# aleju/face-generator

Measured on NVIDIA H100. Metric: 32x32 GAN train images/sec (1 D-iter + 1 G-iter per batch, batch 256/GPU), higher is better.
Workload: dtype f32

## Files before the change

face_generator_b200/csrc/convl.cu:

```cuda
#include "convl.h"

#include "k_conv_tc.h"
#include "k_misc.h"

int convl_dalloc(ConvLEnv& e, float** p, size_t elems) { return fg_dalloc(e.c, *e.allocs, p, elems); }

int ScalePairs::alloc(fg_ctx* c, std::vector<void*>& allocs, int pairs) {
  n = pairs;
  used = 0;
  return fg_dalloc(c, allocs, &base, 2 * (size_t)pairs);
}
int ScalePairs::take(float** pair) {
  if (used == n) {
    fg_set_error("a block of %d FP16 scale pairs is full", n);
    return FG_ERR_UNSUPPORTED;
  }
  *pair = base + 2 * used++;
  return FG_OK;
}
int ScalePairs::reset(fg_ctx* c) const {
  if (!tc_f16(c)) return FG_OK;
  FG_CUDA(cudaMemset2DAsync(base, 2 * sizeof(float), 0, sizeof(float), n, c->stream));
  return FG_OK;
}

namespace {
inline bool tc_f(const fg_ctx* c, const ConvL& L, int B) { return c->conv_impl != FG_CONV_SIMT && tc_conv_eligible(L.geom_k(B)); }
inline bool tc_d(const fg_ctx* c, const ConvL& L, int B) { return c->conv_impl != FG_CONV_SIMT && tc_conv_eligible(L.geom_d(B)); }
inline bool tc_w(const fg_ctx* c, const ConvL& L, int B) { return tc_f(c, L, B) && L.Cout % 128 == 0 && L.geom_k(B).Cin % 64 == 0; }
}

bool convl_tc_fwd(const fg_ctx* c, const ConvL& L) { return tc_f(c, L, 1); }
bool convl_tc_bwd(const fg_ctx* c, const ConvL& L) { return tc_f(c, L, 1) && tc_d(c, L, 1); }

int tc_op_split(fg_ctx* c, TcOp& op, const float* x, int64_t n, bool f16) {
  if (!f16) {
    if (op.split_ready) {
      op.split_ready = false;
      return FG_OK;
    }
    return tc_split(c, x, op.hi, op.lo, n);
  }
  if (op.amax_ready) op.amax_ready = false;
  else FG_TRY(tc_amax(c, x, n, op.s));
  return tc_split_h(c, x, op.hi, op.lo, n, op.s);
}

int convl_alloc(ConvLEnv& e, ConvL& L) {
  const size_t nw = (size_t)L.k * L.k * L.Cout * L.Cin;
  FG_TRY(convl_dalloc(e, &L.Wp, nw));
  FG_TRY(convl_dalloc(e, &L.Wpd, nw));
  if (L.nA) FG_TRY(convl_dalloc(e, &L.bp, L.Cout));
  if (!L.x.s) FG_TRY(convl_dalloc(e, &L.x.s, 2));
  if (!e.dy.s) FG_TRY(convl_dalloc(e, &e.dy.s, 2));
  if (tc_conv_eligible(L.geom_k(e.maxB))) {
    const int K = L.geom_k(e.maxB).Cin;
    const size_t nk = (size_t)L.k * L.k * L.Cout * K, nx = (size_t)e.maxB * L.H * L.H * K;
    FG_TRY(convl_dalloc(e, &L.Wf_hi, nk));
    FG_TRY(convl_dalloc(e, &L.Wf_lo, nk));
    FG_TRY(convl_dalloc(e, &L.x.hi, nx));
    FG_TRY(convl_dalloc(e, &L.x.lo, nx));
    if (L.kpad) {
      FG_TRY(convl_dalloc(e, &L.Wpad, nk));
      FG_TRY(convl_dalloc(e, &L.xpad, nx));
    }
  }
  if (L.need_dgrad && tc_conv_eligible(L.geom_d(e.maxB))) {
    FG_TRY(convl_dalloc(e, &L.Wd_hi, nw));
    FG_TRY(convl_dalloc(e, &L.Wd_lo, nw));
  }
  const int B = e.maxB;
  if (L.pad_out && !(tc_conv_eligible(ConvGeom{B, L.H, L.H, L.Cin, L.pad_out, L.k, 1}) &&
                     tc_conv_eligible(ConvGeom{B, L.H, L.H, L.pad_out, L.Cin, L.k, 1}) && L.Cin % 128 == 0))
    L.pad_out = 0;
  if (L.pad_dy && !(L.x.hi && tc_conv_eligible(ConvGeom{B, L.H, L.H, L.Cin, L.pad_dy, L.k, 1}) && L.Cin % 64 == 0))
    L.pad_dy = 0;
  if (L.pad_out) {
    const size_t nq = (size_t)L.k * L.k * L.pad_out * L.Cin;
    FG_TRY(convl_dalloc(e, &L.Wq_hi, nq));
    FG_TRY(convl_dalloc(e, &L.Wq_lo, nq));
    const size_t nx = (size_t)B * L.H * L.H * L.Cin;
    FG_TRY(convl_dalloc(e, &L.x.hi, nx));
    FG_TRY(convl_dalloc(e, &L.x.lo, nx));
  }
  return FG_OK;
}

int convl_pack(fg_ctx* c, ConvL& L, const float* P) {
  const int KK = L.k * L.k;
  const bool tc_on = c->conv_impl != FG_CONV_SIMT;
  const bool h = tc_on && tc_f16(c) && L.geom_k(1).Cin % 64 == 0 && (L.Cout % 64 == 0 || L.pad_out);
  L.packed_f16 = h;
  if (KK > 1 && tc_on && !L.nA && !L.cA && !L.pad_out && !L.kpad && L.Wf_hi && (L.Wd_hi || !L.need_dgrad) && tc_f(c, L, 1) &&
      (!L.need_dgrad || tc_d(c, L, 1))) {
    if (h) return tc_pack_split_h(c, P + L.w_off, L.Wf_hi, L.Wf_lo, L.Wd_hi, L.Wd_lo, L.Cout, L.Cin, KK);
    return tc_pack_split(c, P + L.w_off, L.Wf_hi, L.Wf_lo, L.Wd_hi, L.Wd_lo, L.Cout, L.Cin, KK);
  }
  FG_TRY(k_pack_weights(c, P + L.w_off, L.Wp, L.need_dgrad ? L.Wpd : nullptr, L.Cout, L.Cin, KK, L.nA, L.nS, L.cA, L.cS));
  if (L.bp) FG_TRY(k_pack_weights(c, P + L.b_off, L.bp, nullptr, L.Cout, 1, 1, L.nA, L.nS, 0, 0));
  if (!tc_on) return FG_OK;
  if (L.kpad && L.Wf_hi) {
    FG_CUDA(cudaMemcpy2DAsync(L.Wpad, L.kpad * sizeof(float), L.Wp, L.Cin * sizeof(float), L.Cin * sizeof(float), L.Cout,
                              cudaMemcpyDeviceToDevice, c->stream));
    if (h) return tc_split_h(c, L.Wpad, L.Wf_hi, L.Wf_lo, (int64_t)L.Cout * L.kpad);
    return tc_split(c, L.Wpad, L.Wf_hi, L.Wf_lo, (int64_t)L.Cout * L.kpad);
  }
  const int64_t nw = (int64_t)KK * L.Cout * L.Cin;
  if (h) {
    if (L.Wf_hi) FG_TRY(tc_split_h(c, L.Wp, L.Wf_hi, L.Wf_lo, nw));
    if (L.Wd_hi) FG_TRY(tc_split_h(c, L.Wpd, L.Wd_hi, L.Wd_lo, nw));
    if (L.pad_out) FG_TRY(k_pack_pad_split_h(c, P + L.w_off, L.Wq_hi, L.Wq_lo, L.Cout, L.pad_out, L.Cin, KK));
    return FG_OK;
  }
  if (L.Wf_hi) FG_TRY(tc_split(c, L.Wp, L.Wf_hi, L.Wf_lo, nw));
  if (L.Wd_hi) FG_TRY(tc_split(c, L.Wpd, L.Wd_hi, L.Wd_lo, nw));
  if (L.pad_out) FG_TRY(k_pack_pad_split(c, P + L.w_off, L.Wq_hi, L.Wq_lo, L.Cout, L.pad_out, L.Cin, KK));
  return FG_OK;
}

int convl_fwd(ConvLEnv& e, ConvL& L, const float* in, const float* P, float* out, int B) {
  fg_ctx* c = e.c;
  const ConvGeom g = L.geom(B);
  const float* bias = L.bp ? L.bp : P + L.b_off;
  const bool h = L.packed_f16;
  const float* os = h ? L.x.s + 1 : nullptr;
  if (L.pad_out && c->conv_impl != FG_CONV_SIMT) {
    FG_TRY(tc_op_split(c, L.x, in, (int64_t)B * L.H * L.H * L.Cin, h));
    {
      ScopedTimer t(c, L.tf);
      FG_TRY(tc_conv_fwd(c, L.x.hi, L.x.lo, L.Wq_hi, L.Wq_lo, nullptr, e.ga, ConvGeom{B, L.H, L.H, L.Cin, L.pad_out, L.k, 1}, 0,
                         nullptr, nullptr, h, os));
    }
    return k_compact_bias(c, e.ga, bias, out, (int64_t)B * L.H * L.H, L.Cout, L.pad_out);
  }
  if (tc_f(c, L, B)) {
    const ConvGeom gk = L.geom_k(B);
    if (L.kpad) {
      FG_CUDA(cudaMemcpy2DAsync(L.xpad, L.kpad * sizeof(float), in, L.Cin * sizeof(float), L.Cin * sizeof(float), (size_t)B * L.H * L.H,
                                cudaMemcpyDeviceToDevice, c->stream));
      in = L.xpad;
    }
    FG_TRY(tc_op_split(c, L.x, in, (int64_t)B * L.H * L.H * gk.Cin, h));
    ScopedTimer t(c, L.tf);
    return tc_conv_fwd(c, L.x.hi, L.x.lo, L.Wf_hi, L.Wf_lo, bias, out, gk, 0, nullptr, nullptr, h, os);
  }
  ScopedTimer t(c, L.tf);
  if (c->edge_impl && k_edge_eligible(g)) return k_conv_edge(c, in, L.Wp, bias, out, g);
  return k_small_eligible(g) ? k_conv_small(c, in, L.Wp, bias, out, g) : k_conv_simt(c, in, L.Wp, bias, out, g);
}

int convl_bwd(ConvLEnv& e, ConvL& L, const float* in, const float* dy, float* G, float* din, int B) {
  fg_ctx* c = e.c;
  const ConvGeom g = L.geom(B), gd = L.geom_d(B);
  const bool w_tc = G && tc_w(c, L, B), d_tc = din && tc_d(c, L, B);
  const bool h = L.packed_f16;
  float* sdy = L.sdy ? L.sdy : e.dy.s;
  const bool split_ready = e.dy.split_ready, amax_ready = e.dy.amax_ready, bias_ready = e.dy.bias_ready;
  e.dy.split_ready = e.dy.amax_ready = e.dy.bias_ready = false;
  const float *osy = h ? sdy + 1 : nullptr, *osx = h ? L.x.s + 1 : nullptr;
  const bool tc_on = c->conv_impl != FG_CONV_SIMT;
  const int64_t P = (int64_t)B * L.H * L.H;
  if (h && !amax_ready && (w_tc || d_tc || (G && tc_on && (L.pad_out || L.pad_dy)))) FG_TRY(tc_amax(c, dy, P * L.Cout, sdy));
  if (w_tc || d_tc) {
    if (h) FG_TRY(tc_split_h(c, dy, e.dy.hi, e.dy.lo, P * L.Cout, sdy));
    else if (!split_ready) FG_TRY(tc_split(c, dy, e.dy.hi, e.dy.lo, P * L.Cout));
  }
  if (G && tc_on && L.pad_out) {
    if (h) FG_TRY(k_pad_split_h(c, dy, e.pad.hi, e.pad.lo, P, L.Cout, L.pad_out, sdy));
    else FG_TRY(k_pad_split(c, dy, e.pad.hi, e.pad.lo, P, L.Cout, L.pad_out));
    {
      ScopedTimer t(c, L.tw);
      FG_TRY(tc_conv_wgrad(c, e.pad.hi, e.pad.lo, L.x.hi, L.x.lo, e.ws, ConvGeom{B, L.H, L.H, L.pad_out, L.Cin, L.k, 1}, h, osy, osx));
    }
    FG_TRY(k_unpack_wgrad_swapped(c, e.ws, G + L.w_off, L.Cout, L.pad_out, L.Cin, L.k * L.k));
    if (!bias_ready) FG_TRY(k_colsum_add(c, dy, G + L.b_off, P, L.Cout, 0, 0));
  } else if (G && tc_on && L.pad_dy && !w_tc) {
    if (h) FG_TRY(k_pad_split_h(c, dy, e.pad.hi, e.pad.lo, P, L.Cout, L.pad_dy, sdy));
    else FG_TRY(k_pad_split(c, dy, e.pad.hi, e.pad.lo, P, L.Cout, L.pad_dy));
    {
      ScopedTimer t(c, L.tw);
      FG_TRY(tc_conv_wgrad(c, L.x.hi, L.x.lo, e.pad.hi, e.pad.lo, e.ws, ConvGeom{B, L.H, L.H, L.Cin, L.pad_dy, L.k, 1}, h, osy, osx));
    }
    FG_TRY(k_unpack_wgrad_pad(c, e.ws, G + L.w_off, L.Cout, L.pad_dy, L.Cin, L.k * L.k));
    if (!bias_ready) FG_TRY(k_colsum_add(c, dy, G + L.b_off, P, L.Cout, 0, 0));
  } else if (G) {
    const int64_t koff = L.kpad && w_tc ? (int64_t)L.Cout * L.Cin : 0;
    {
      ScopedTimer t(c, L.tw);
      if (w_tc) FG_TRY(tc_conv_wgrad(c, L.x.hi, L.x.lo, e.dy.hi, e.dy.lo, e.ws + koff, L.geom_k(B), h, osy, osx));
      else if (k_small_eligible(g)) FG_TRY(k_wgrad_small(c, in, dy, e.ws, g));
      else FG_TRY(k_wgrad_simt(c, in, dy, e.ws, g));
    }
    if (koff)
      FG_CUDA(cudaMemcpy2DAsync(e.ws, L.Cin * sizeof(float), e.ws + koff, L.kpad * sizeof(float), L.Cin * sizeof(float), L.Cout,
                                cudaMemcpyDeviceToDevice, c->stream));
    FG_TRY(k_unpack_wgrad(c, e.ws, G + L.w_off, L.Cout, L.Cin, L.k * L.k, L.nA, L.nS, L.cA, L.cS));
    if (!bias_ready) FG_TRY(k_colsum_add(c, dy, G + L.b_off, P, L.Cout, L.nA, L.nS));
  }
  if (din) {
    ScopedTimer t(c, L.td);
    if (d_tc) return tc_conv_fwd(c, e.dy.hi, e.dy.lo, L.Wd_hi, L.Wd_lo, nullptr, din, gd, 0, nullptr, nullptr, h, osy);
    if (c->edge_impl && k_edge_eligible(gd)) return k_conv_edge(c, dy, L.Wpd, nullptr, din, gd);
    return k_small_eligible(gd) ? k_conv_small(c, dy, L.Wpd, nullptr, din, gd) : k_conv_simt(c, dy, L.Wpd, nullptr, din, gd);
  }
  return FG_OK;
}

bool upsl_tc(const fg_ctx* c, const UpsL& U) {
  return c->conv_impl != FG_CONV_SIMT && tc_conv_eligible(U.geom(1)) && U.Cout % 128 == 0 && U.Cin % 64 == 0;
}

int upsl_alloc(ConvLEnv& e, UpsL& U) {
  const size_t nw25 = (size_t)25 * U.Cout * U.Cin, nw36 = (size_t)36 * U.Cout * U.Cin;
  FG_TRY(convl_dalloc(e, &U.Wp, nw25));
  FG_TRY(convl_dalloc(e, &U.Wpd, nw25));
  FG_TRY(convl_dalloc(e, &U.Wf_hi, nw36));
  FG_TRY(convl_dalloc(e, &U.Wf_lo, nw36));
  FG_TRY(convl_dalloc(e, &U.Wd_hi, nw36));
  FG_TRY(convl_dalloc(e, &U.Wd_lo, nw36));
  FG_TRY(convl_dalloc(e, &U.Wx_hi, nw25));
  FG_TRY(convl_dalloc(e, &U.Wx_lo, nw25));
  const size_t nx = (size_t)e.maxB * (U.H / 2) * (U.H / 2) * U.Cin;
  FG_TRY(convl_dalloc(e, &U.x.hi, nx));
  FG_TRY(convl_dalloc(e, &U.x.lo, nx));
  if (!U.x.s) FG_TRY(convl_dalloc(e, &U.x.s, 2));
  return FG_OK;
}

int upsl_pack(fg_ctx* c, UpsL& U, const float* P) {
  const float* W = P + U.w_off;
  if (!upsl_tc(c, U)) return k_pack_weights(c, W, U.Wp, U.Wpd, U.Cout, U.Cin, 25, 0, 0, 0, 0);
  if (tc_f16(c)) FG_TRY(tc_pack_collapsed_h(c, W, U.Wf_hi, U.Wf_lo, U.Wd_hi, U.Wd_lo, U.Cout, U.Cin));
  else FG_TRY(tc_pack_collapsed(c, W, U.Wf_hi, U.Wf_lo, U.Wd_hi, U.Wd_lo, U.Cout, U.Cin));
  if (c->conv_impl == FG_CONV_TC_DENSE) FG_TRY(tc_pack_split(c, W, U.Wx_hi, U.Wx_lo, nullptr, nullptr, U.Cout, U.Cin, 25));
  return FG_OK;
}

int upsl_fwd(ConvLEnv& e, UpsL& U, const float* h, const float* P, float* z, int B, int* parts) {
  fg_ctx* c = e.c;
  const ConvGeom g = U.geom(B);
  const bool want = parts && *parts;
  if (parts) *parts = 0;
  const float* bias = P + U.b_off;
  if (!upsl_tc(c, U)) {
    ScopedTimer t(c, U.tf);
    return k_conv_simt(c, h, U.Wp, bias, z, g);
  }
  const bool f16 = tc_f16(c);
  FG_TRY(tc_op_split(c, U.x, h, (int64_t)B * (U.H / 2) * (U.H / 2) * U.Cin, f16));
  ScopedTimer t(c, U.tf);
  float* st = want && c->bn_epilogue ? c->bn_parts : nullptr;
  const bool dense = c->conv_impl == FG_CONV_TC_DENSE;
  return tc_conv_fwd(c, U.x.hi, U.x.lo, dense ? U.Wx_hi : U.Wf_hi, dense ? U.Wx_lo : U.Wf_lo, bias, z, g, dense ? 1 : 2, st,
                     st ? parts : nullptr, f16, f16 ? U.x.s + 1 : nullptr);
}

int upsl_bwd(ConvLEnv& e, UpsL& U, TcOp& dy, const float* h, const float* dz, float* G, float* dh, int B, bool* pooled) {
  fg_ctx* c = e.c;
  const ConvGeom g = U.geom(B);
  float* dW = G + U.w_off;
  *pooled = upsl_tc(c, U);
  if (!*pooled) {
    {
      ScopedTimer t(c, U.tw);
      FG_TRY(k_wgrad_simt(c, h, dz, e.ws, g));
    }
    FG_TRY(k_unpack_wgrad(c, e.ws, dW, U.Cout, U.Cin, 25, 0, 0, 0, 0));
    ScopedTimer t(c, U.td);
    return k_conv_simt(c, dz, U.Wpd, nullptr, dh, ConvGeom{B, U.H, U.H, U.Cout, U.Cin, 5, 1});
  }
  const bool f16 = tc_f16(c);
  FG_TRY(tc_op_split(c, dy, dz, (int64_t)B * U.H * U.H * U.Cout, f16));
  const float *sy = f16 ? dy.s + 1 : nullptr, *sx = f16 ? U.x.s + 1 : nullptr;
  if (f16 && U.tb && (c->bwd_merge == 2 ? tc_bwd_pair_eligible(c, g) : c->bwd_merge == 1 && tc_bwd_pair_pays(c, g))) {
    {
      ScopedTimer t(c, U.tb);
      FG_TRY(tc_conv_bwd_ups(c, U.x.hi, U.x.lo, dy.hi, dy.lo, U.Wd_hi, U.Wd_lo, e.ws, dh, g, sy, sx));
    }
    return tc_combine_collapsed_wgrad(c, e.ws, dW, U.Cout, U.Cin);
  }
  {
    ScopedTimer t(c, U.tw);
    FG_TRY(tc_conv_wgrad(c, U.x.hi, U.x.lo, dy.hi, dy.lo, e.ws, g, f16, sy, sx));
  }
  FG_TRY(tc_combine_collapsed_wgrad(c, e.ws, dW, U.Cout, U.Cin));
  ScopedTimer t(c, U.td);
  return tc_conv_dgrad_ups(c, dy.hi, dy.lo, U.Wd_hi, U.Wd_lo, dh, g, f16, sy);
}
```

face_generator_b200/csrc/convl.h:

```cpp
#pragma once
#include <vector>

#include "fg_internal.h"

inline bool tc_f16(const fg_ctx* c) { return c->mma_f16 && c->conv_impl == FG_CONV_TC_COLLAPSED; }

struct AmaxInto {
  fg_ctx* c;
  AmaxInto(fg_ctx* c_, TcOp& op) : AmaxInto(c_, op.s, &op.amax_ready) {}
  AmaxInto(fg_ctx* c_, float* pair, bool* done) : c(c_) {
    if (tc_f16(c)) {
      c->amax_out = reinterpret_cast<unsigned*>(pair);
      c->amax_done = done;
    }
  }
  ~AmaxInto() { c->amax_out = nullptr; }
};

int tc_op_split(fg_ctx* c, TcOp& op, const float* x, int64_t n, bool f16);

inline int pack_key(const fg_ctx* c) { return c->conv_impl | (c->mma_f16 << 4); }
int convl_dalloc(ConvLEnv& e, float** p, size_t elems);
int convl_alloc(ConvLEnv& e, ConvL& L);
bool convl_tc_fwd(const fg_ctx* c, const ConvL& L);
bool convl_tc_bwd(const fg_ctx* c, const ConvL& L);
int convl_pack(fg_ctx* c, ConvL& L, const float* P);
int convl_fwd(ConvLEnv& e, ConvL& L, const float* in, const float* P, float* out, int B);
int convl_bwd(ConvLEnv& e, ConvL& L, const float* in, const float* dy, float* G, float* din, int B);

bool upsl_tc(const fg_ctx* c, const UpsL& U);
int upsl_alloc(ConvLEnv& e, UpsL& U);
int upsl_pack(fg_ctx* c, UpsL& U, const float* P);
int upsl_fwd(ConvLEnv& e, UpsL& U, const float* h, const float* P, float* z, int B, int* parts = nullptr);
int upsl_bwd(ConvLEnv& e, UpsL& U, TcOp& dy, const float* h, const float* dz, float* G, float* dh, int B, bool* pooled);

int gen_alloc(ConvLEnv& e, UpsGen& G, const GenDesc& d);
int gen_pack(fg_ctx* c, UpsGen& G, NetPair& p);
int gen_forward(ConvLEnv& e, UpsGen& G, NetPair& p, const float* noise, int B, bool training);
int gen_backward(ConvLEnv& e, UpsGen& G, NetPair& p, const float* dy, float* dnoise);
void gen_debug_rows(const UpsGen& G, std::vector<DebugTensor>& rows);
```

face_generator_b200/csrc/fg_internal.h:

```cpp
#pragma once
#include <cuda_runtime.h>
#include <cstdint>
#include <cstdio>
#include <deque>
#include <functional>
#include <initializer_list>
#include <map>
#include <string>
#include <vector>

#include "fg_b200.h"

void fg_set_error(const char* fmt, ...);

#define FG_CUDA(call)                                                                               \
  do {                                                                                              \
    cudaError_t e__ = (call);                                                                       \
    if (e__ != cudaSuccess) {                                                                       \
      fg_set_error("%s:%d: %s -> %s", __FILE__, __LINE__, #call, cudaGetErrorString(e__));          \
      return FG_ERR_CUDA;                                                                           \
    }                                                                                               \
  } while (0)
#define FG_TRY(call)                  \
  do {                                \
    int r__ = (call);                 \
    if (r__ != FG_OK) return r__;     \
  } while (0)
#define FG_REQUIRE(cond, ...)         \
  do {                                \
    if (!(cond)) {                    \
      fg_set_error(__VA_ARGS__);      \
      return FG_ERR_INVALID;          \
    }                                 \
  } while (0)
#define LAUNCH_CHECK(c)                 \
  do {                                  \
    (c)->launches++;                    \
    FG_CUDA(cudaGetLastError());        \
  } while (0)
inline int grid_for(int64_t n, int block, int cap = 132 * 16) {
  int64_t g = (n + block - 1) / block;
  if (g > cap) g = cap;
  if (g < 1) g = 1;
  return (int)g;
}
#define GRID_STRIDE(i, n) \
  for (int64_t i = blockIdx.x * (int64_t)blockDim.x + threadIdx.x; i < (n); i += (int64_t)gridDim.x * blockDim.x)

constexpr int kMaskPerSample = 1984;
constexpr int kNoiseDim = 100;
constexpr int kSmallMaxParts = 2048;
constexpr int kGradTail = 8;
constexpr int kOptRedRows = 132 * 2;

struct ConvGeom {
  int B, H, W, Cin, Cout, k, ups;
};

struct GLayout {
  int64_t L1W, L1b, a1, C1W, C1b, g1, be1, a2, C2W, C2b, g2, be2, a3, C3W, C3b, total;
};
struct DLayout {
  int64_t cW[4], cb[4], ca[4], L1W, L1b, a5, L2W, L2b, a6, L3W, L3b, total;
};
GLayout make_g_layout(int C, int side);
DLayout make_d_layout(int C);

struct DeviceStats {
  float loss_D, loss_G;
  int conf[4];
  int trained_D;
  int t_D, t_G;
  float acc_D;
  int acc_count, acc_head;
  float step_D, step_G;
  int do_train_D, do_train_G;
};
constexpr int kAccHistMax = 1024;
constexpr int kBnState = 768;

struct StepGraph {
  std::vector<uint8_t> key;
  cudaGraphExec_t exec = nullptr;
  int64_t launches = 0;
  bool failed = false;
};

struct NetPair {
  int64_t nG = 0, nD = 0;
  float *PG = nullptr, *PD = nullptr, *gG = nullptr, *gD = nullptr;
  float *tailG = nullptr, *tailD = nullptr;
  float *mG = nullptr, *vG = nullptr, *mD = nullptr, *vD = nullptr;
  float* bnG = nullptr;
  DeviceStats* dstats = nullptr;
  DeviceStats* hstats = nullptr;
  float* acc_hist = nullptr;
  bool G_packed = false, D_packed = false;
  std::vector<StepGraph> graphs;
  const char* optim_timer[2] = {nullptr, nullptr};
};

struct ScalePairs {
  float* base = nullptr;
  int n = 0, used = 0;
  int alloc(fg_ctx* c, std::vector<void*>& allocs, int pairs);
  int take(float** pair);
  int reset(fg_ctx* c) const;
};

struct TcOp {
  float *hi = nullptr, *lo = nullptr;
  float* s = nullptr;
  bool split_ready = false, amax_ready = false, bias_ready = false;
};
struct ConvL {
  int Cin = 0, Cout = 0, k = 1, H = 1;
  int64_t w_off = 0, b_off = 0;
  int cA = 0, cS = 0;
  int nA = 0, nS = 0;
  float *Wp = nullptr, *Wpd = nullptr;
  float* bp = nullptr;
  float *Wf_hi = nullptr, *Wf_lo = nullptr, *Wd_hi = nullptr, *Wd_lo = nullptr;
  TcOp x;
  float* sdy = nullptr;
  int kpad = 0;
  float *xpad = nullptr, *Wpad = nullptr;
  bool packed_f16 = false;
  int pad_out = 0, pad_dy = 0;
  float *Wq_hi = nullptr, *Wq_lo = nullptr;
  bool need_dgrad = true;
  const char *tf = "", *td = "", *tw = "";
  ConvGeom geom(int B) const { return ConvGeom{B, H, H, Cin, Cout, k, 1}; }
  ConvGeom geom_k(int B) const { return ConvGeom{B, H, H, kpad ? kpad : Cin, Cout, k, 1}; }
  ConvGeom geom_d(int B) const { return ConvGeom{B, H, H, Cout, Cin, k, 1}; }
};

struct UpsL {
  int Cin = 0, Cout = 0, H = 0;
  int64_t w_off = 0, b_off = 0;
  float *Wp = nullptr, *Wpd = nullptr;
  float *Wf_hi = nullptr, *Wf_lo = nullptr, *Wd_hi = nullptr, *Wd_lo = nullptr;
  float *Wx_hi = nullptr, *Wx_lo = nullptr;
  TcOp x;
  const char *tf = "", *td = "", *tw = "", *tb = nullptr;
  ConvGeom geom(int B) const { return ConvGeom{B, H, H, Cin, Cout, 5, 2}; }
};

struct ConvLEnv {
  fg_ctx* c = nullptr;
  int maxB = 0;
  std::vector<void*>* allocs = nullptr;
  float *ga = nullptr;
  TcOp dy;
  TcOp pad;
  float* ws = nullptr;
};

struct GenDesc {
  int side;
  const char* prefix;
  int l1_kpad;
  bool bwd_merge;
};

struct UpsGen {
  int S = 32, C = 3;
  GLayout gl;
  ConvL GL1, GC3;
  UpsL GU[2];
  ScalePairs pairs;
  float* sdz[2] = {nullptr, nullptr};
  float *noise = nullptr, *z0 = nullptr, *h0 = nullptr, *z1 = nullptr, *h1 = nullptr, *z2 = nullptr, *h2 = nullptr,
        *z3 = nullptr, *y = nullptr;
  float *dz3 = nullptr, *dfull = nullptr, *dz2 = nullptr, *dz1 = nullptr, *dz0 = nullptr;
  float *bn_mean[2] = {nullptr, nullptr}, *bn_istd[2] = {nullptr, nullptr}, *bn_mg = nullptr;
  int B = 0;
  bool train = true, valid = false;
  int pack_key = -1;
  std::deque<std::string> names;
  const char *t_bn2_finalize = nullptr, *t_bn2_stats = nullptr, *t_bn2_apply = nullptr, *t_bn2_bwd_reduce = nullptr,
             *t_bn2_bwd_apply = nullptr;
};

struct TimerRec {
  double ms = 0;
  int64_t launches = 0;
  std::vector<std::pair<cudaEvent_t, cudaEvent_t>> pending;
};

struct fg_ctx {
  int device = 0, maxB = 0, C = 3;
  cudaStream_t stream = nullptr;
  bool own_stream = true;
  int64_t launches = 0;
  int conv_impl = FG_CONV_TC_COLLAPSED;
  int sm_count = 132;
  int opt_D = 0, opt_G = 0;
  float sgd_mom_D = 0.f, sgd_mom_G = 0.f;
  DLayout dl;
  std::vector<void*> allocs;
  NetPair net;
  float *ownPG = nullptr, *ownPD = nullptr, *ownGG = nullptr, *ownGD = nullptr;
  float* tail_sep = nullptr;
  float* small_ws = nullptr;
  float* wgrad_ws = nullptr;
  size_t wgrad_ws_elems = 0;
  float* splitk_ws = nullptr;
  size_t splitk_ws_elems = 0;
  double* red_ws = nullptr;
  size_t red_ws_elems = 0;
  double* red_ws_opt = nullptr;
  unsigned* red_ticket = nullptr;
  double* bn_slice_acc = nullptr;
  float* bn_parts = nullptr;
  int edge_impl = 1;
  int bn_epilogue = 1;
  int mma_f16 = 1;
  float* lop_sx = nullptr;
  float* lop_sy = nullptr;
  unsigned* amax_out = nullptr;
  bool* amax_done = nullptr;
  double* bn_acc = nullptr;
  int D_B = 0;
  bool D_train = true, D_fwd_valid = false;
  float *D_x = nullptr, *D_z[4] = {nullptr, nullptr, nullptr, nullptr}, *D_p[4] = {nullptr, nullptr, nullptr, nullptr};
  float *D_zl1 = nullptr, *D_hl1 = nullptr, *D_zl2 = nullptr, *D_hl2 = nullptr, *D_logit = nullptr, *D_out = nullptr;
  float* D_masks = nullptr;
  float D_drop_scale = 2.0f, D_spatial_eval = 0.8f;
  float *D_dlogit = nullptr, *D_dh = nullptr, *D_dzl = nullptr, *D_dz = nullptr, *D_dp = nullptr, *D_dx = nullptr;
  float* D_targets = nullptr;
  float* stage_pinned = nullptr;
  size_t stage_pinned_bytes = 0;
  float* io_dev = nullptr;
  size_t io_dev_elems = 0;
  float* io_dev2 = nullptr;
  float *in_real = nullptr, *in_noiseD = nullptr, *in_noiseG = nullptr, *in_masksD = nullptr, *in_masksG = nullptr;
  float* scratch[8] = {nullptr, nullptr, nullptr, nullptr, nullptr, nullptr, nullptr, nullptr};
  size_t scratch_elems[8] = {0, 0, 0, 0, 0, 0, 0, 0};
  void* nccl_comm = nullptr;
  int world = 1, rank = 0;
  int dp_overlap = 1;
  int reserve_sms = 0;
  int bwd_merge = 1, bwd_merge_ctas = 0;
  int* bwd_claim = nullptr;
  int use_graph = 1, graph_epoch = 0;
  uint64_t* seed_dev = nullptr;
  cudaStream_t comm_stream = nullptr;
  cudaEvent_t ev_fork = nullptr, ev_join = nullptr;
  bool debug_keep = false;
  int keep_B = 0;
  float* keep_D[8] = {nullptr, nullptr, nullptr, nullptr, nullptr, nullptr, nullptr, nullptr};
  cudaEvent_t events[16] = {};
  bool timing = false;
  std::map<std::string, TimerRec> timers;
  ConvLEnv env;
  UpsGen G;
  ConvL Dc[4], DL1, DL2;
  ScalePairs D_pairs;
};

struct ScopedTimer {
  fg_ctx* c;
  TimerRec* rec = nullptr;
  cudaEvent_t e0 = nullptr, e1 = nullptr;
  ScopedTimer(fg_ctx* c_, const char* name) : c(c_) {
    if (c->timing && name) {
      rec = &c->timers[name];
      cudaEventCreate(&e0);
      cudaEventCreate(&e1);
      cudaEventRecord(e0, c->stream);
    }
  }
  ~ScopedTimer() {
    if (rec) {
      cudaEventRecord(e1, c->stream);
      rec->pending.emplace_back(e0, e1);
    }
  }
};

int k_fill(fg_ctx* c, float* p, float v, int64_t n);
int k_nchw_to_nhwc(fg_ctx* c, const float* src, float* dst, int B, int C, int HW);
int k_nhwc_to_nchw(fg_ctx* c, const float* src, float* dst, int B, int C, int HW);
int k_pack_weights(fg_ctx* c, const float* W, float* Wp, float* Wpd, int N, int Cc, int KK, int nA, int nS, int cA,
                   int cS);
int k_unpack_wgrad(fg_ctx* c, const float* dWp, float* dW, int N, int Cc, int KK, int nA, int nS, int cA, int cS);
int k_colsum_add(fg_ctx* c, const float* X, float* out, int64_t P, int N, int nA, int nS);
int k_prelu_fwd(fg_ctx* c, const float* z, const float* slope, float* h, int64_t n);
int k_prelu_bwd(fg_ctx* c, const float* dh, const float* z, const float* slope, float* dz, float* dslope, int B, int H,
                int W, int C, int pool);
int k_bn_stats(fg_ctx* c, const float* z, double* acc2C, int64_t P, int C);
bool k_bn4_ok(int C);
int k_bn_stats4(fg_ctx* c, const float* z, double* acc, int64_t P, int C);
int k_bn_bwd_reduce4(fg_ctx* c, const float* dh, const float* z, const float* mean, const float* istd, const float* gamma,
                     const float* beta, const float* slope, double* acc, float* dslope, int64_t P, int C);
int k_bn_finalize(fg_ctx* c, double* acc2C, float* mean, float* istd, float* run_mean, float* run_var, int64_t P,
                  int C);
int k_bn_finalize_parts(fg_ctx* c, const float* part, int nparts, float* mean, float* istd, float* run_mean, float* run_var,
                        int64_t P, int C);
int k_bn_eval_prep(fg_ctx* c, const float* run_mean, const float* run_var, float* mean, float* istd, int C);
int k_bn_prelu_apply(fg_ctx* c, const float* z, const float* mean, const float* istd, const float* gamma,
                     const float* beta, const float* slope, float* h, int64_t P, int C, float* hi = nullptr,
                     float* lo = nullptr);
int k_bn_prelu_bwd_reduce(fg_ctx* c, const float* dh, const float* z, const float* mean, const float* istd,
                          const float* gamma, const float* beta, const float* slope, double* acc2C, float* dslope,
                          int B, int H, int W, int C, int pool);
int k_bn_bwd_finalize(fg_ctx* c, double* acc2C, float* mg2C, float* dgamma, float* dbeta, int64_t P, int C);
int k_bn_prelu_bwd_apply(fg_ctx* c, const float* dh, const float* z, const float* mean, const float* istd,
                         const float* gamma, const float* beta, const float* slope, const float* mg2C, float* dz,
                         int B, int H, int W, int C, int pool, float* hi = nullptr, float* lo = nullptr,
                         float* dbias = nullptr);
int k_sigmoid_fwd(fg_ctx* c, const float* z, float* y, int64_t n);
int k_sigmoid_bwd(fg_ctx* c, const float* dy, const float* y, float* dz, int64_t n);
int k_masks_generate(fg_ctx* c, float* masks, int B, uint64_t seed, float p_spatial, float p_drop,
                     const uint64_t* seed_dev = nullptr);
int k_set_u64(fg_ctx* c, uint64_t* dst, uint64_t v);
int k_d_act_pool_fwd(fg_ctx* c, const float* z, const float* slope, const float* masks, int moff, float eval_scale,
                     float* p, int B, int H, int W, int C, float* hi = nullptr, float* lo = nullptr);
int k_d_act_pool_bwd(fg_ctx* c, const float* dp, const float* z, const float* slope, const float* masks, int moff,
                     float eval_scale, float* dz, float* dslope, int B, int H, int W, int C, float* hi = nullptr,
                     float* lo = nullptr, float* dbias = nullptr);
int k_lin_act_drop_fwd(fg_ctx* c, const float* z, const float* slope, const float* masks, int moff, float scale,
                       float* h, int B, int N);
int k_lin_act_drop_bwd(fg_ctx* c, const float* dh, const float* z, const float* slope, const float* masks, int moff,
                       float scale, float* dz, float* dslope, int B, int N);
int k_sigmoid_bce(fg_ctx* c, const float* logit, float* out, float* dlogit, float* loss_out, float* tail4, int B,
                  int n_ones);
int k_bce_fwd(fg_ctx* c, const float* x, const float* t, int n, float* loss_out);
int k_bce_bwd(fg_ctx* c, const float* x, const float* t, int n, float* dx);
int k_sigmoid_grad_mul(fg_ctx* c, const float* dout, const float* out, float* dlogit, int n);
int k_penalty_loss(fg_ctx* c, const float* p, int64_t n, float l1, float l2, float* loss_inout);
int k_gate_and_prep(fg_ctx* c, DeviceStats* st, float* acc_hist, int net, const fg_hyper* h, const float* tail4, int B,
                    float world);
int k_gemv_fwd(fg_ctx* c, const float* x, const float* w, const float* bias, float* out, int B, int K);
int k_gemv_dgrad(fg_ctx* c, const float* dy, const float* w, float* dx, int B, int K);
int k_gemv_wgrad_add(fg_ctx* c, const float* x, const float* dy, float* dw, float* db, int B, int K);
int k_adam(fg_ctx* c, float* p, const float* g, float* m, float* v, int64_t n, float beta1, float beta2, float eps,
           float l1_grad, float l2, float clampv, float grad_scale, const float* step_dev, const int* flag_dev,
           float step_host, float* g_out);
int k_optim_update(fg_ctx* c, int mode, float* p, float* g, float* m, float* v, int64_t n, float beta1, float beta2, float eps,
                   float mom, float l1_grad, float l2, float clampv, float grad_scale, const float* step_dev,
                   const int* flag_dev, const int* t_dev);

int k_conv_simt(fg_ctx* c, const float* in, const float* Wp, const float* bias, float* out, ConvGeom g);
int k_wgrad_simt(fg_ctx* c, const float* in, const float* dY, float* dWp, ConvGeom g);
bool k_small_eligible(const ConvGeom& g);
int k_conv_small(fg_ctx* c, const float* in, const float* Wp, const float* bias, float* out, ConvGeom g);
int k_wgrad_small(fg_ctx* c, const float* in, const float* dY, float* dWp, ConvGeom g);

bool k_edge_eligible(const ConvGeom& g);
int k_conv_edge(fg_ctx* c, const float* in, const float* Wp, const float* bias, float* out, ConvGeom g);

inline int red_check(fg_ctx* c, int64_t rows, int64_t n) {
  if (rows * n > (int64_t)c->red_ws_elems) {
    fg_set_error("ordered reduction of %lld x %lld partials exceeds its workspace", (long long)rows, (long long)n);
    return FG_ERR_UNSUPPORTED;
  }
  return FG_OK;
}
int k_splitk_reduce(fg_ctx* c, const float* parts, int splits, int64_t n, float* out);

int tc_init(fg_ctx* c);
void tc_destroy(fg_ctx* c);

int net_alloc(fg_ctx* c);
void net_free(fg_ctx* c);
int net_pack_D(fg_ctx* c);
int net_D_forward(fg_ctx* c, const float* x_nhwc, int B, bool training, const fg_hyper* h);
int net_D_backward(fg_ctx* c, const float* dlogit_dev, bool want_wgrad, bool want_dx);
int net_train_step(fg_ctx* c, const fg_hyper* h, int B, const float* real_nchw_dev, const float* noiseD_dev,
                   const float* noiseG_dev, const float* masksD_dev, const float* masksG_dev, uint64_t seed,
                   bool allow_graph = false);
int net_allreduce(fg_ctx* c, float* buf, int64_t n);
int net_broadcast(fg_ctx* c, void* buf, size_t bytes);
int net_group(bool start);

int fg_dalloc(fg_ctx* c, std::vector<void*>& allocs, float** p, size_t n);
int pair_alloc(fg_ctx* c, std::vector<void*>& allocs, NetPair& p, int64_t nG, int64_t nD, bool bn);
void pair_clear_graphs(NetPair& p);
void pair_free(NetPair& p);
int pair_zero_grads(fg_ctx* c, NetPair& p, int net);
int pair_allreduce_grads(fg_ctx* c, NetPair& p, int net);
int pair_gate(fg_ctx* c, NetPair& p, int net, const fg_hyper* h, int B, float world);
int pair_optim(fg_ctx* c, NetPair& p, int net, const fg_hyper* h, float grad_scale);
int pair_broadcast(fg_ctx* c, NetPair& p);
int pair_step_stats(fg_ctx* c, const NetPair& p, fg_step_stats* stats);
int pair_set_params(fg_ctx* c, NetPair& p, int net, const float* src);
int pair_get_params(fg_ctx* c, const NetPair& p, int net, float* dst);
int pair_get_grads(fg_ctx* c, const NetPair& p, int net, float* dst);
int pair_set_adam_state(fg_ctx* c, NetPair& p, int net, const float* m, const float* v, int t);
int pair_get_adam_state(fg_ctx* c, const NetPair& p, int net, float* m, float* v, int* t);
int pair_set_bn_state(fg_ctx* c, NetPair& p, const float* src);
int pair_get_bn_state(fg_ctx* c, const NetPair& p, float* dst);
int net_graph_run(fg_ctx* c, NetPair& p, int B, const fg_hyper* h, std::initializer_list<const void*> inputs, uint64_t seed,
                  const std::function<int()>& body, bool allow_graph);

bool fg_is_dev(const void* p);
int fg_to_dev(fg_ctx* c, const float* p, size_t n, float* staging, const float** out);
int fg_to_user(fg_ctx* c, float* dst, const float* src_dev, size_t n);
struct DebugTensor {
  const char* name;
  const float* p;
  int64_t per;
  int B;
};
int64_t debug_tensor_copy(fg_ctx* c, const char* what, const DebugTensor* ents, size_t n_ents, const char* name, float* dst,
                          int64_t max_elems);

int dataset_check_feed(const fg_dataset* d, const fg_ctx* c, const char* what);
int dataset_draw_gather(fg_dataset* d, uint64_t seed, int B, int size, float* out_dev);
int dataset_draw_gather_c2f(fg_dataset* d, uint64_t seed, int B, int coarse_size, float* fine, float* coarse, float* diff);
int noise_uniform_dev(fg_ctx* c, uint64_t seed, int64_t n, float* out_dev);
```

face_generator_b200/csrc/gen.cu:

```cuda
#include "convl.h"

GLayout make_g_layout(int C, int side) {
  const int64_t n0 = 128 * (side / 4) * (side / 4);
  GLayout L;
  int64_t o = 0;
  L.L1W = o; o += n0 * kNoiseDim;
  L.L1b = o; o += n0;
  L.a1 = o; o += 1;
  L.C1W = o; o += 256 * 128 * 25;
  L.C1b = o; o += 256;
  L.g1 = o; o += 256;
  L.be1 = o; o += 256;
  L.a2 = o; o += 1;
  L.C2W = o; o += 128 * 256 * 25;
  L.C2b = o; o += 128;
  L.g2 = o; o += 128;
  L.be2 = o; o += 128;
  L.a3 = o; o += 1;
  L.C3W = o; o += (int64_t)C * 128 * 9;
  L.C3b = o; o += C;
  L.total = o;
  return L;
}

int gen_alloc(ConvLEnv& e, UpsGen& G, const GenDesc& d) {
  fg_ctx* c = e.c;
  const int S = d.side, C = c->C;
  G.S = S;
  G.C = C;
  G.gl = make_g_layout(C, S);
  const GLayout& gl = G.gl;
  auto timer = [&](const char* name) {
    G.names.push_back(std::string(d.prefix) + name);
    return G.names.back().c_str();
  };
  FG_TRY(G.pairs.alloc(c, *e.allocs, 8));
  ConvL& L1 = G.GL1;
  L1.Cin = kNoiseDim; L1.Cout = 128 * (S / 4) * (S / 4); L1.k = 1; L1.H = 1;
  L1.w_off = gl.L1W; L1.b_off = gl.L1b;
  L1.nA = 128; L1.nS = (S / 4) * (S / 4);
  L1.kpad = d.l1_kpad;
  L1.tf = timer("G.L1.fwd"); L1.td = timer("G.L1.dgrad"); L1.tw = timer("G.L1.wgrad");
  ConvL& C3 = G.GC3;
  C3.Cin = 128; C3.Cout = C; C3.k = 3; C3.H = S;
  C3.w_off = gl.C3W; C3.b_off = gl.C3b;
  C3.tf = timer("G.C3.fwd"); C3.td = timer("G.C3.dgrad"); C3.tw = timer("G.C3.wgrad");
  for (ConvL* L : {&L1, &C3}) {
    FG_TRY(G.pairs.take(&L->x.s));
    FG_TRY(G.pairs.take(&L->sdy));
    FG_TRY(convl_alloc(e, *L));
  }
  static const char* uf[2] = {"G.C1.fwd", "G.C2.fwd"};
  static const char* ud[2] = {"G.C1.dgrad", "G.C2.dgrad"};
  static const char* uw[2] = {"G.C1.wgrad", "G.C2.wgrad"};
  static const char* ub[2] = {"G.C1.wgrad+dgrad", "G.C2.wgrad+dgrad"};
  const int ci[2] = {128, 256}, co[2] = {256, 128}, hs[2] = {S / 2, S};
  const int64_t wo[2] = {gl.C1W, gl.C2W}, bo[2] = {gl.C1b, gl.C2b};
  for (int i = 0; i < 2; ++i) {
    UpsL& U = G.GU[i];
    U.Cin = ci[i]; U.Cout = co[i]; U.H = hs[i];
    U.w_off = wo[i]; U.b_off = bo[i];
    U.tf = timer(uf[i]); U.td = timer(ud[i]); U.tw = timer(uw[i]);
    U.tb = d.bwd_merge ? timer(ub[i]) : nullptr;
    FG_TRY(G.pairs.take(&U.x.s));
    FG_TRY(G.pairs.take(&G.sdz[i]));
    FG_TRY(upsl_alloc(e, U));
  }
  G.t_bn2_finalize = timer("G.bn2.finalize");
  G.t_bn2_stats = timer("hbm.G.bn2.stats");
  G.t_bn2_apply = timer("hbm.G.bn2.apply");
  G.t_bn2_bwd_reduce = timer("hbm.G.bn2.bwd_reduce");
  G.t_bn2_bwd_apply = timer("hbm.G.bn2.bwd_apply");
  const size_t B = e.maxB, n0 = L1.Cout, n1 = (size_t)256 * (S / 2) * (S / 2), n2 = (size_t)128 * S * S, n3 = (size_t)C * S * S;
  for (auto [p, n] : {std::pair<float**, size_t>{&G.noise, kNoiseDim}, {&G.z0, n0}, {&G.h0, n0}, {&G.z1, n1}, {&G.h1, n1},
                      {&G.z2, n2}, {&G.h2, n2}, {&G.z3, n3}, {&G.y, n3}, {&G.dz3, n3},
                      {&G.dfull, (size_t)256 * S * S},
                      {&G.dz2, n2}, {&G.dz1, n1}, {&G.dz0, n0}})
    FG_TRY(convl_dalloc(e, p, B * n));
  for (int i = 0; i < 2; ++i) {
    FG_TRY(convl_dalloc(e, &G.bn_mean[i], co[i]));
    FG_TRY(convl_dalloc(e, &G.bn_istd[i], co[i]));
  }
  return convl_dalloc(e, &G.bn_mg, 512);
}

int gen_pack(fg_ctx* c, UpsGen& G, NetPair& p) {
  if (p.G_packed && G.pack_key == pack_key(c)) return FG_OK;
  FG_TRY(convl_pack(c, G.GL1, p.PG));
  for (int i = 0; i < 2; ++i) FG_TRY(upsl_pack(c, G.GU[i], p.PG));
  FG_TRY(convl_pack(c, G.GC3, p.PG));
  p.G_packed = true;
  G.pack_key = pack_key(c);
  return FG_OK;
}

namespace {
int bn_stats(fg_ctx* c, UpsGen& G, NetPair& p, int i, const float* z, int B, bool training, int parts, const char* t_finalize,
             const char* t_stats) {
  const int Cc = G.GU[i].Cout;
  const int64_t P = (int64_t)B * G.GU[i].H * G.GU[i].H;
  float *rm = p.bnG + (i == 0 ? 0 : 512), *rv = rm + Cc;
  if (!training) return k_bn_eval_prep(c, rm, rv, G.bn_mean[i], G.bn_istd[i], Cc);
  if (parts) {
    ScopedTimer tm(c, t_finalize);
    return k_bn_finalize_parts(c, c->bn_parts, parts, G.bn_mean[i], G.bn_istd[i], rm, rv, P, Cc);
  }
  {
    ScopedTimer tm(c, t_stats);
    FG_TRY(k_bn_stats(c, z, c->bn_acc, P, Cc));
  }
  return k_bn_finalize(c, c->bn_acc, G.bn_mean[i], G.bn_istd[i], rm, rv, P, Cc);
}
}

int gen_forward(ConvLEnv& e, UpsGen& G, NetPair& p, const float* noise, int B, bool training) {
  fg_ctx* c = e.c;
  FG_REQUIRE(B >= 1 && B <= e.maxB, "G forward: batch %d out of range [1,%d]", B, e.maxB);
  FG_TRY(gen_pack(c, G, p));
  const GLayout& L = G.gl;
  const float* P = p.PG;
  const int S = G.S;
  if (noise != G.noise)
    FG_CUDA(cudaMemcpyAsync(G.noise, noise, sizeof(float) * B * kNoiseDim, cudaMemcpyDeviceToDevice, c->stream));
  G.B = B;
  G.train = training;
  FG_TRY(G.pairs.reset(c));
  FG_TRY(convl_fwd(e, G.GL1, G.noise, P, G.z0, B));
  {
    AmaxInto am(c, G.GU[0].x);
    FG_TRY(k_prelu_fwd(c, G.z0, P + L.a1, G.h0, (int64_t)B * G.GL1.Cout));
  }
  int parts = training ? 1 : 0;
  FG_TRY(upsl_fwd(e, G.GU[0], G.h0, P, G.z1, B, &parts));
  FG_TRY(bn_stats(c, G, p, 0, G.z1, B, training, parts, nullptr, nullptr));
  UpsL& C2 = G.GU[1];
  C2.x.split_ready = training && upsl_tc(c, C2) && !tc_f16(c);
  {
    AmaxInto am(c, C2.x);
    FG_TRY(k_bn_prelu_apply(c, G.z1, G.bn_mean[0], G.bn_istd[0], P + L.g1, P + L.be1, P + L.a2, G.h1,
                            (int64_t)B * (S / 2) * (S / 2), 256, C2.x.split_ready ? C2.x.hi : nullptr,
                            C2.x.split_ready ? C2.x.lo : nullptr));
  }
  parts = training ? 1 : 0;
  FG_TRY(upsl_fwd(e, C2, G.h1, P, G.z2, B, &parts));
  FG_TRY(bn_stats(c, G, p, 1, G.z2, B, training, parts, G.t_bn2_finalize, G.t_bn2_stats));
  {
    ScopedTimer tm(c, G.t_bn2_apply);
    FG_TRY(k_bn_prelu_apply(c, G.z2, G.bn_mean[1], G.bn_istd[1], P + L.g2, P + L.be2, P + L.a3, G.h2, (int64_t)B * S * S, 128));
  }
  FG_TRY(convl_fwd(e, G.GC3, G.h2, P, G.z3, B));
  FG_TRY(k_sigmoid_fwd(c, G.z3, G.y, (int64_t)B * S * S * G.C));
  G.valid = true;
  return FG_OK;
}

int gen_backward(ConvLEnv& e, UpsGen& G, NetPair& p, const float* dy, float* dnoise) {
  fg_ctx* c = e.c;
  if (!G.valid || !G.train) {
    fg_set_error("G backward needs a preceding training-mode G forward");
    return FG_ERR_STATE;
  }
  const GLayout& L = G.gl;
  const float* P = p.PG;
  float* g = p.gG;
  const int B = G.B, S = G.S, h = S / 2;
  FG_TRY(G.pairs.reset(c));
  FG_TRY(k_sigmoid_bwd(c, dy, G.y, G.dz3, (int64_t)B * S * S * G.C));
  FG_TRY(convl_bwd(e, G.GC3, G.h2, G.dz3, g, G.dfull, B));
  {
    ScopedTimer tm(c, G.t_bn2_bwd_reduce);
    FG_TRY(k_bn_prelu_bwd_reduce(c, G.dfull, G.z2, G.bn_mean[1], G.bn_istd[1], P + L.g2, P + L.be2, P + L.a3, c->bn_acc,
                                 g + L.a3, B, S, S, 128, 0));
  }
  FG_TRY(k_bn_bwd_finalize(c, c->bn_acc, G.bn_mg, g + L.g2, g + L.be2, (int64_t)B * S * S, 128));
  const bool tf32 = !tc_f16(c);
  TcOp dz2{e.dy.hi, e.dy.lo, G.sdz[1]};
  dz2.split_ready = upsl_tc(c, G.GU[1]) && tf32;
  {
    ScopedTimer tm(c, G.t_bn2_bwd_apply);
    AmaxInto am(c, dz2);
    FG_TRY(k_bn_prelu_bwd_apply(c, G.dfull, G.z2, G.bn_mean[1], G.bn_istd[1], P + L.g2, P + L.be2, P + L.a3, G.bn_mg, G.dz2,
                                B, S, S, 128, 0, dz2.split_ready ? dz2.hi : nullptr, dz2.split_ready ? dz2.lo : nullptr,
                                g + L.C2b));
  }
  bool pooled = false;
  FG_TRY(upsl_bwd(e, G.GU[1], dz2, G.h1, G.dz2, g, G.dfull, B, &pooled));
  FG_TRY(k_bn_prelu_bwd_reduce(c, G.dfull, G.z1, G.bn_mean[0], G.bn_istd[0], P + L.g1, P + L.be1, P + L.a2, c->bn_acc,
                               g + L.a2, B, h, h, 256, pooled ? 0 : 1));
  FG_TRY(k_bn_bwd_finalize(c, c->bn_acc, G.bn_mg, g + L.g1, g + L.be1, (int64_t)B * h * h, 256));
  TcOp dz1{e.dy.hi, e.dy.lo, G.sdz[0]};
  dz1.split_ready = upsl_tc(c, G.GU[0]) && tf32 && pooled;
  {
    AmaxInto am(c, dz1);
    FG_TRY(k_bn_prelu_bwd_apply(c, G.dfull, G.z1, G.bn_mean[0], G.bn_istd[0], P + L.g1, P + L.be1, P + L.a2, G.bn_mg, G.dz1,
                                B, h, h, 256, pooled ? 0 : 1, dz1.split_ready ? dz1.hi : nullptr,
                                dz1.split_ready ? dz1.lo : nullptr, g + L.C1b));
  }
  FG_TRY(upsl_bwd(e, G.GU[0], dz1, G.h0, G.dz1, g, G.dfull, B, &pooled));
  {
    AmaxInto am(c, G.GL1.sdy, &e.dy.amax_ready);
    FG_TRY(k_prelu_bwd(c, G.dfull, G.z0, P + L.a1, G.dz0, g + L.a1, B, S / 4, S / 4, 128, pooled ? 0 : 1));
  }
  return convl_bwd(e, G.GL1, G.noise, G.dz0, g, dnoise, B);
}

void gen_debug_rows(const UpsGen& G, std::vector<DebugTensor>& rows) {
  const int64_t n0 = G.GL1.Cout, n1 = 256 * (G.S / 2) * (G.S / 2), n2 = 128 * G.S * G.S, n3 = (int64_t)G.C * G.S * G.S;
  const int B = G.B;
  for (const DebugTensor& r : {DebugTensor{"G.z0", G.z0, n0, B}, {"G.h0", G.h0, n0, B}, {"G.z1", G.z1, n1, B},
                               {"G.h1", G.h1, n1, B}, {"G.z2", G.z2, n2, B}, {"G.h2", G.h2, n2, B}, {"G.z3", G.z3, n3, B},
                               {"G.y", G.y, n3, B}, {"G.dz2", G.dz2, n2, B}, {"G.dz1", G.dz1, n1, B}, {"G.dz0", G.dz0, n0, B},
                               {"G.bn_mean1", G.bn_mean[0], 256, 1}, {"G.bn_istd1", G.bn_istd[0], 256, 1},
                               {"G.bn_mean2", G.bn_mean[1], 128, 1}, {"G.bn_istd2", G.bn_istd[1], 128, 1}})
    rows.push_back({r.name, G.valid ? r.p : nullptr, r.per, r.B});
}
```

face_generator_b200/csrc/k_conv_edge.cu:

```cuda
#include <cuda.h>

#include <algorithm>

#include "fg_internal.h"
#include "k_conv_tc.h"

namespace {
constexpr int kW = 32;

__device__ __forceinline__ uint32_t smem_u32(const void* p) { return (uint32_t)__cvta_generic_to_shared(p); }
__device__ __forceinline__ void mbar_init(uint64_t* bar, uint32_t count) {
  asm volatile("mbarrier.init.shared::cta.b64 [%0], %1;" ::"r"(smem_u32(bar)), "r"(count));
}
__device__ __forceinline__ void mbar_expect_tx(uint64_t* bar, uint32_t bytes) {
  asm volatile("mbarrier.arrive.expect_tx.shared::cta.b64 _, [%0], %1;" ::"r"(smem_u32(bar)), "r"(bytes) : "memory");
}
__device__ __forceinline__ void mbar_wait(uint64_t* bar, uint32_t parity) {
  const uint32_t addr = smem_u32(bar);
  uint32_t ok;
  do {
    asm volatile(
        "{\n\t.reg .pred p;\n\t"
        "mbarrier.try_wait.parity.shared::cta.b64 p, [%1], %2;\n\t"
        "selp.b32 %0, 1, 0, p;\n\t}"
        : "=r"(ok)
        : "r"(addr), "r"(parity)
        : "memory");
  } while (!ok);
}
__device__ __forceinline__ float4 lds128(uint32_t addr) {
  float4 v;
  asm volatile("ld.shared.v4.f32 {%0, %1, %2, %3}, [%4];" : "=f"(v.x), "=f"(v.y), "=f"(v.z), "=f"(v.w) : "r"(addr));
  return v;
}
__device__ __forceinline__ float2 lds64(uint32_t addr) {
  float2 v;
  asm volatile("ld.shared.v2.f32 {%0, %1}, [%2];" : "=f"(v.x), "=f"(v.y) : "r"(addr));
  return v;
}
__device__ __forceinline__ void tma_load_4d(void* dst, const CUtensorMap* map, uint64_t* bar, int c0, int c1, int c2, int c3) {
  asm volatile(
      "cp.async.bulk.tensor.4d.shared::cluster.global.mbarrier::complete_tx::bytes [%0], [%1, {%3, %4, %5, %6}], [%2];"
      ::"r"(smem_u32(dst)), "l"(map), "r"(smem_u32(bar)), "r"(c0), "r"(c1), "r"(c2), "r"(c3)
      : "memory");
}

constexpr int kRedRows = 4;
template <int VEC>
constexpr uint32_t red_tile_bytes() { return (kRedRows + 2) * (kW + 2) * 32 * VEC * 4; }

template <int NS, int VEC>
__global__ void __launch_bounds__(256, 1) conv_reduce_kernel(const __grid_constant__ CUtensorMap tmap, const float* __restrict__ Wp,
                                                             const float* __restrict__ bias, float* __restrict__ out, int H,
                                                             int nunits) {
  constexpr int C = 32 * VEC;
  constexpr int PX = NS == 1 ? 16 : 4;
  constexpr uint32_t kTile = red_tile_bytes<VEC>();
  extern __shared__ uint8_t smem_raw[];
  uint8_t* smem = reinterpret_cast<uint8_t*>((reinterpret_cast<uintptr_t>(smem_raw) + 127) & ~(uintptr_t)127);
  uint64_t* full = reinterpret_cast<uint64_t*>(smem + 2 * kTile);
  const int warp = threadIdx.x >> 5, lane = threadIdx.x & 31;
  const int strips = H / kRedRows;
  if (threadIdx.x == 0) {
    mbar_init(full + 0, 1);
    mbar_init(full + 1, 1);
    asm volatile("fence.mbarrier_init.release.cluster;" ::: "memory");
  }
  __syncthreads();
  auto issue = [&](int unit, int buf) {
    const int b = unit / strips, y0 = (unit - b * strips) * kRedRows;
    asm volatile("fence.proxy.async.shared::cta;" ::: "memory");
    mbar_expect_tx(full + buf, kTile);
    tma_load_4d(smem + buf * kTile, &tmap, full + buf, 0, -1, y0 - 1, b);
  };
  if (threadIdx.x == 0 && (int)blockIdx.x < nunits) issue(blockIdx.x, 0);
  float w[9][NS][VEC];
#pragma unroll
  for (int t = 0; t < 9; ++t)
#pragma unroll
    for (int n = 0; n < NS; ++n)
#pragma unroll
      for (int j = 0; j < VEC; ++j) w[t][n][j] = Wp[(t * NS + n) * C + lane * VEC + j];
  float bv = 0.f;
  if (bias && (lane & 15) < PX * NS) bv = bias[(lane & 15) % NS];
  const int row = warp >> 1, xh = (warp & 1) * 16;
  int it = 0;
  for (int unit = blockIdx.x; unit < nunits; unit += gridDim.x, ++it) {
    const int buf = it & 1;
    if (threadIdx.x == 0 && unit + (int)gridDim.x < nunits) issue(unit + gridDim.x, buf ^ 1);
    mbar_wait(full + buf, (it >> 1) & 1);
    const uint32_t tile = smem_u32(smem + buf * kTile) + (uint32_t)lane * VEC * 4;
    const int b = unit / strips, y = (unit - b * strips) * kRedRows + row;
#pragma unroll 1
    for (int g = 0; g < 16 / PX; ++g) {
      const int x0 = xh + g * PX;
      float acc[PX][NS];
#pragma unroll
      for (int i = 0; i < PX; ++i)
#pragma unroll
        for (int n = 0; n < NS; ++n) acc[i][n] = 0.f;
#pragma unroll
      for (int j = 0; j < PX + 2; ++j) {
        float v[3][VEC];
#pragma unroll
        for (int dy = 0; dy < 3; ++dy) {
          const uint32_t ad = tile + (uint32_t)(((row + dy) * (kW + 2) + x0 + j) * C) * 4;
          if (VEC == 4) {
            const float4 q = lds128(ad);
            v[dy][0] = q.x; v[dy][1 % VEC] = q.y; v[dy][2 % VEC] = q.z; v[dy][3 % VEC] = q.w;
          } else {
            const float2 q = lds64(ad);
            v[dy][0] = q.x; v[dy][1 % VEC] = q.y;
          }
        }
#pragma unroll
        for (int dy = 0; dy < 3; ++dy)
#pragma unroll
          for (int k = 0; k < VEC; ++k)
#pragma unroll
            for (int dx = 0; dx < 3; ++dx) {
              const int i = j - dx;
              if (i < 0 || i >= PX) continue;
#pragma unroll
              for (int n = 0; n < NS; ++n) acc[i][n] = fmaf(v[dy][k], w[dy * 3 + dx][n][k], acc[i][n]);
            }
      }
      float r[16];
#pragma unroll
      for (int k = 0; k < 16; ++k) r[k] = k < PX * NS ? acc[k / NS][k % NS] : 0.f;
#pragma unroll
      for (int sft = 8; sft >= 1; sft >>= 1) {
        const bool up = (lane & sft) != 0;
#pragma unroll
        for (int k = 0; k < sft; ++k) {
          const float send = up ? r[k] : r[k + sft], keep = up ? r[k + sft] : r[k];
          r[k] = keep + __shfl_xor_sync(0xffffffffu, send, sft);
        }
      }
      const float tot = r[0] + __shfl_xor_sync(0xffffffffu, r[0], 16);
      if (lane < PX * NS) out[((size_t)(b * H + y) * kW + x0) * NS + lane] = tot + bv;
    }
    __syncthreads();
  }
}

constexpr int kExpRows = 8;
template <int CS, int N>
__global__ void __launch_bounds__(256, 1) conv_expand_kernel(const float* __restrict__ in, const float* __restrict__ Wp,
                                                             const float* __restrict__ bias, float* __restrict__ out, int H,
                                                             int nunits) {
  constexpr int RW = (kW + 2) * 4;
  constexpr int ROWF = kW * CS;
  constexpr int NPF = ((kExpRows + 2) * ROWF + 255) / 256;
  __shared__ __align__(16) float tile[2][(kExpRows + 2) * RW];
  const int warp = threadIdx.x >> 5, lane = threadIdx.x & 31;
  const int strips = H / kExpRows;
  for (int i = threadIdx.x; i < 2 * (kExpRows + 2) * RW; i += 256) (&tile[0][0])[i] = 0.f;
  const int n4 = (N == 128 ? lane : (lane & 15)) * 4;
  float w[9][CS][4];
#pragma unroll
  for (int t = 0; t < 9; ++t)
#pragma unroll
    for (int c = 0; c < CS; ++c)
#pragma unroll
      for (int j = 0; j < 4; ++j) w[t][c][j] = Wp[((size_t)t * N + n4 + j) * CS + c];
  float4 b4 = make_float4(0.f, 0.f, 0.f, 0.f);
  if (bias) b4 = make_float4(bias[n4], bias[n4 + 1], bias[n4 + 2], bias[n4 + 3]);
  float pf[NPF];
  auto prefetch = [&](int unit) {
    const int b = unit / strips, y0 = (unit - b * strips) * kExpRows;
#pragma unroll
    for (int i = 0; i < NPF; ++i) {
      const int idx = threadIdx.x + 256 * i;
      const int r = idx / ROWF, off = idx - r * ROWF, gy = y0 - 1 + r;
      pf[i] = (r < kExpRows + 2 && gy >= 0 && gy < H) ? in[((size_t)(b * H + gy) * kW) * CS + off] : 0.f;
    }
  };
  auto stash = [&](int buf) {
#pragma unroll
    for (int i = 0; i < NPF; ++i) {
      const int idx = threadIdx.x + 256 * i;
      const int r = idx / ROWF, off = idx - r * ROWF;
      if (r < kExpRows + 2) tile[buf][r * RW + (off / CS + 1) * 4 + off % CS] = pf[i];
    }
  };
  __syncthreads();
  if ((int)blockIdx.x < nunits) {
    prefetch(blockIdx.x);
    stash(0);
  }
  __syncthreads();
  constexpr int STEP = N == 128 ? 2 : 4;
  const int xoff = N == 128 ? 0 : 2 * (lane >> 4);
  int it = 0;
  for (int unit = blockIdx.x; unit < nunits; unit += gridDim.x, ++it) {
    const int buf = it & 1;
    const bool more = unit + (int)gridDim.x < nunits;
    if (more) prefetch(unit + gridDim.x);
    const int b = unit / strips, y = (unit - b * strips) * kExpRows + warp;
    const float4* t0 = reinterpret_cast<const float4*>(&tile[buf][warp * RW]);
    float* orow = out + ((size_t)(b * H + y) * kW) * N + n4;
#pragma unroll 1
    for (int xb = 0; xb < kW; xb += STEP) {
      const int x = xb + xoff;
      float4 a0 = b4, a1 = b4;
#pragma unroll
      for (int dy = 0; dy < 3; ++dy) {
        float4 col[4];
#pragma unroll
        for (int j = 0; j < 4; ++j) col[j] = t0[dy * (kW + 2) + x + j];
#pragma unroll
        for (int dx = 0; dx < 3; ++dx)
#pragma unroll
          for (int c = 0; c < CS; ++c) {
            const float v0 = c == 0 ? col[dx].x : (c == 1 ? col[dx].y : (c == 2 ? col[dx].z : col[dx].w));
            const float v1 = c == 0 ? col[dx + 1].x : (c == 1 ? col[dx + 1].y : (c == 2 ? col[dx + 1].z : col[dx + 1].w));
            const float* wp = w[dy * 3 + dx][c];
            a0.x = fmaf(v0, wp[0], a0.x); a1.x = fmaf(v1, wp[0], a1.x);
            a0.y = fmaf(v0, wp[1], a0.y); a1.y = fmaf(v1, wp[1], a1.y);
            a0.z = fmaf(v0, wp[2], a0.z); a1.z = fmaf(v1, wp[2], a1.z);
            a0.w = fmaf(v0, wp[3], a0.w); a1.w = fmaf(v1, wp[3], a1.w);
          }
      }
      *reinterpret_cast<float4*>(orow + (size_t)x * N) = a0;
      *reinterpret_cast<float4*>(orow + (size_t)(x + 1) * N) = a1;
    }
    if (more) stash(buf ^ 1);
    __syncthreads();
  }
}

template <int NS, int VEC>
int launch_reduce(fg_ctx* c, const float* in, const float* Wp, const float* bias, float* out, const ConvGeom& g) {
  CUtensorMap tmap;
  FG_TRY(tc_encode_nhwc_box(&tmap, in, 32 * VEC, g.W, g.H, g.B, 32 * VEC, kW + 2, kRedRows + 2, 1));
  const int nunits = g.B * (g.H / kRedRows);
  const size_t smem = 2 * (size_t)red_tile_bytes<VEC>() + 64 + 128;
  static bool attr_done = false;
  if (!attr_done) {
    FG_CUDA(cudaFuncSetAttribute(conv_reduce_kernel<NS, VEC>, cudaFuncAttributeMaxDynamicSharedMemorySize, (int)smem));
    attr_done = true;
  }
  conv_reduce_kernel<NS, VEC><<<std::min(nunits, c->sm_count), 256, smem, c->stream>>>(tmap, Wp, bias, out, g.H, nunits);
  LAUNCH_CHECK(c);
  return FG_OK;
}
template <int CS, int N>
int launch_expand(fg_ctx* c, const float* in, const float* Wp, const float* bias, float* out, const ConvGeom& g) {
  const int nunits = g.B * (g.H / kExpRows);
  conv_expand_kernel<CS, N><<<std::min(nunits, c->sm_count), 256, 0, c->stream>>>(in, Wp, bias, out, g.H, nunits);
  LAUNCH_CHECK(c);
  return FG_OK;
}
}

bool k_edge_eligible(const ConvGeom& g) {
  if (!(g.ups == 1 && g.k == 3 && g.W == kW && g.H % 8 == 0 && g.H >= 8)) return false;
  const bool reduce = (g.Cout == 1 || g.Cout == 3) && (g.Cin == 64 || g.Cin == 128);
  const bool expand = (g.Cin == 1 || g.Cin == 3 || g.Cin == 4) && (g.Cout == 64 || g.Cout == 128);
  return reduce || expand;
}

int k_conv_edge(fg_ctx* c, const float* in, const float* Wp, const float* bias, float* out, ConvGeom g) {
  if (g.Cout <= 3) {
    if (g.Cout == 3 && g.Cin == 128) return launch_reduce<3, 4>(c, in, Wp, bias, out, g);
    if (g.Cout == 3 && g.Cin == 64) return launch_reduce<3, 2>(c, in, Wp, bias, out, g);
    if (g.Cout == 1 && g.Cin == 128) return launch_reduce<1, 4>(c, in, Wp, bias, out, g);
    if (g.Cout == 1 && g.Cin == 64) return launch_reduce<1, 2>(c, in, Wp, bias, out, g);
  } else {
#define EXP(CS_)                                                                 \
  if (g.Cin == CS_) {                                                            \
    if (g.Cout == 128) return launch_expand<CS_, 128>(c, in, Wp, bias, out, g); \
    if (g.Cout == 64) return launch_expand<CS_, 64>(c, in, Wp, bias, out, g);   \
  }
    EXP(1) EXP(3) EXP(4)
#undef EXP
  }
  fg_set_error("k_conv_edge: unsupported shape %d -> %d", g.Cin, g.Cout);
  return FG_ERR_UNSUPPORTED;
}
```

face_generator_b200/csrc/k_elem.cu:

```cuda
#include <cmath>

#include "fg_internal.h"
#include "k_ordered.cuh"

__device__ __forceinline__ int perm_idx(int j, int A, int S) {
  if (A == 0) return j;
  return (j % S) * A + (j / S);
}

__device__ __forceinline__ double warp_sum(double v) {
#pragma unroll
  for (int o = 16; o > 0; o >>= 1) v += __shfl_xor_sync(0xffffffffu, v, o);
  return v;
}
__device__ __forceinline__ double block_sum(double v) {
  __shared__ double red[32];
  __syncthreads();
  v = warp_sum(v);
  if ((threadIdx.x & 31) == 0) red[threadIdx.x >> 5] = v;
  __syncthreads();
  if (threadIdx.x < 32) {
    v = threadIdx.x < (blockDim.x + 31) / 32 ? red[threadIdx.x] : 0.0;
    v = warp_sum(v);
  }
  return v;
}

__device__ __forceinline__ void amax_commit(unsigned* amax, float m) {
  if (!amax) return;
#pragma unroll
  for (int o = 16; o > 0; o >>= 1) m = fmaxf(m, __shfl_xor_sync(0xffffffffu, m, o));
  if ((threadIdx.x & 31) == 0 && m > 0.f) {
    const unsigned bits = __float_as_uint(m);
    if (bits > *reinterpret_cast<volatile unsigned*>(amax)) atomicMax(amax, bits);
  }
}
__device__ __forceinline__ float amax4(float m, float a, float b, float c, float d) {
  return fmaxf(fmaxf(m, fmaxf(fabsf(a), fabsf(b))), fmaxf(fabsf(c), fabsf(d)));
}
static inline unsigned* take_amax(fg_ctx* c) {
  unsigned* p = c->amax_out;
  if (p) *c->amax_done = true;
  return p;
}

__global__ void fill_kernel(float* p, float v, int64_t n) {
  for (int64_t i = blockIdx.x * (int64_t)blockDim.x + threadIdx.x; i < n; i += (int64_t)gridDim.x * blockDim.x) p[i] = v;
}
int k_fill(fg_ctx* c, float* p, float v, int64_t n) {
  if (n <= 0) return FG_OK;
  fill_kernel<<<grid_for(n, 256), 256, 0, c->stream>>>(p, v, n);
  LAUNCH_CHECK(c);
  return FG_OK;
}

__global__ void nchw_to_nhwc_kernel(const float* __restrict__ src, float* __restrict__ dst, int B, int C, int HW) {
  const int64_t n = (int64_t)B * C * HW;
  for (int64_t i = blockIdx.x * (int64_t)blockDim.x + threadIdx.x; i < n; i += (int64_t)gridDim.x * blockDim.x) {
    const int ch = (int)(i % C);
    const int64_t r = i / C;
    const int p = (int)(r % HW);
    const int b = (int)(r / HW);
    dst[i] = src[((int64_t)b * C + ch) * HW + p];
  }
}
__global__ void nhwc_to_nchw_kernel(const float* __restrict__ src, float* __restrict__ dst, int B, int C, int HW) {
  const int64_t n = (int64_t)B * C * HW;
  for (int64_t i = blockIdx.x * (int64_t)blockDim.x + threadIdx.x; i < n; i += (int64_t)gridDim.x * blockDim.x) {
    const int p = (int)(i % HW);
    const int64_t r = i / HW;
    const int ch = (int)(r % C);
    const int b = (int)(r / C);
    dst[i] = src[((int64_t)b * HW + p) * C + ch];
  }
}
int k_nchw_to_nhwc(fg_ctx* c, const float* src, float* dst, int B, int C, int HW) {
  nchw_to_nhwc_kernel<<<grid_for((int64_t)B * C * HW, 256), 256, 0, c->stream>>>(src, dst, B, C, HW);
  LAUNCH_CHECK(c);
  return FG_OK;
}
int k_nhwc_to_nchw(fg_ctx* c, const float* src, float* dst, int B, int C, int HW) {
  nhwc_to_nchw_kernel<<<grid_for((int64_t)B * C * HW, 256), 256, 0, c->stream>>>(src, dst, B, C, HW);
  LAUNCH_CHECK(c);
  return FG_OK;
}

__global__ void pack_weights_kernel(const float* __restrict__ W, float* __restrict__ Wp, float* __restrict__ Wpd, int N,
                                    int Cc, int KK, int nA, int nS, int cA, int cS) {
  const int64_t total = (int64_t)N * Cc * KK;
  for (int64_t i = blockIdx.x * (int64_t)blockDim.x + threadIdx.x; i < total; i += (int64_t)gridDim.x * blockDim.x) {
    const int t = (int)(i % KK);
    const int64_t r = i / KK;
    const int ch = (int)(r % Cc);
    const int n = (int)(r / Cc);
    const int n2 = perm_idx(n, nA, nS), c2 = perm_idx(ch, cA, cS);
    const float w = W[i];
    if (Wp) Wp[((int64_t)t * N + n2) * Cc + c2] = w;
    if (Wpd) Wpd[((int64_t)(KK - 1 - t) * Cc + c2) * N + n2] = w;
  }
}
int k_pack_weights(fg_ctx* c, const float* W, float* Wp, float* Wpd, int N, int Cc, int KK, int nA, int nS, int cA,
                   int cS) {
  pack_weights_kernel<<<grid_for((int64_t)N * Cc * KK, 256), 256, 0, c->stream>>>(W, Wp, Wpd, N, Cc, KK, nA, nS, cA, cS);
  LAUNCH_CHECK(c);
  return FG_OK;
}
__global__ void unpack_wgrad_kernel(const float* __restrict__ dWp, float* __restrict__ dW, int N, int Cc, int KK, int nA,
                                    int nS, int cA, int cS) {
  const int64_t total = (int64_t)N * Cc * KK;
  for (int64_t i = blockIdx.x * (int64_t)blockDim.x + threadIdx.x; i < total; i += (int64_t)gridDim.x * blockDim.x) {
    const int t = (int)(i % KK);
    const int64_t r = i / KK;
    const int ch = (int)(r % Cc);
    const int n = (int)(r / Cc);
    const int n2 = perm_idx(n, nA, nS), c2 = perm_idx(ch, cA, cS);
    dW[i] += dWp[((int64_t)t * N + n2) * Cc + c2];
  }
}
int k_unpack_wgrad(fg_ctx* c, const float* dWp, float* dW, int N, int Cc, int KK, int nA, int nS, int cA, int cS) {
  unpack_wgrad_kernel<<<grid_for((int64_t)N * Cc * KK, 256), 256, 0, c->stream>>>(dWp, dW, N, Cc, KK, nA, nS, cA, cS);
  LAUNCH_CHECK(c);
  return FG_OK;
}

__global__ void colsum_kernel(const float* __restrict__ X, float* __restrict__ out, int64_t P, int N, int nA, int nS,
                              int64_t rows_per_block, double* __restrict__ ws, unsigned* __restrict__ ticket) {
  __shared__ double sm[8][33];
  const int col = blockIdx.x * 32 + threadIdx.x;
  const int64_t r0 = blockIdx.y * rows_per_block;
  const int64_t r1 = min(P, r0 + rows_per_block);
  double s = 0;
  if (col < N)
    for (int64_t r = r0 + threadIdx.y; r < r1; r += 8) s += X[r * N + col];
  sm[threadIdx.y][threadIdx.x] = s;
  __syncthreads();
  if (threadIdx.y == 0 && col < N) {
    double t = 0;
#pragma unroll
    for (int i = 0; i < 8; ++i) t += sm[i][threadIdx.x];
    const int j = nA == 0 ? col : (col % nA) * nS + (col / nA);
    ws[(int64_t)blockIdx.y * N + j] = t;
  }
  if (ordered_last_block(ticket)) {
    for (int j = threadIdx.y * blockDim.x + threadIdx.x; j < N; j += blockDim.x * blockDim.y)
      out[j] += (float)ordered_sum(ws, gridDim.y, N, j);
    ordered_release(ticket);
  }
}
int k_colsum_add(fg_ctx* c, const float* X, float* out, int64_t P, int N, int nA, int nS) {
  int gy = (int)std::min<int64_t>(256, (P + 255) / 256);
  if (gy < 1) gy = 1;
  const int64_t rpb = (P + gy - 1) / gy;
  dim3 grid((N + 31) / 32, gy), block(32, 8);
  FG_TRY(red_check(c, gy, N));
  colsum_kernel<<<grid, block, 0, c->stream>>>(X, out, P, N, nA, nS, rpb, c->red_ws, c->red_ticket);
  LAUNCH_CHECK(c);
  return FG_OK;
}

__global__ void prelu_fwd_kernel(const float* __restrict__ z, const float* __restrict__ slope, float* __restrict__ h,
                                 int64_t n, unsigned* __restrict__ amax) {
  const float a = *slope;
  float am = 0.f;
  for (int64_t i = blockIdx.x * (int64_t)blockDim.x + threadIdx.x; i < n; i += (int64_t)gridDim.x * blockDim.x) {
    const float v = z[i];
    const float o = v > 0.f ? v : a * v;
    h[i] = o;
    am = fmaxf(am, fabsf(o));
  }
  amax_commit(amax, am);
}
int k_prelu_fwd(fg_ctx* c, const float* z, const float* slope, float* h, int64_t n) {
  prelu_fwd_kernel<<<grid_for(n, 256), 256, 0, c->stream>>>(z, slope, h, n, take_amax(c));
  LAUNCH_CHECK(c);
  return FG_OK;
}

__device__ __forceinline__ float load_dh(const float* __restrict__ dh, int b, int y, int x, int ch, int H, int W, int C,
                                         int pool) {
  if (!pool) return dh[(((int64_t)b * H + y) * W + x) * C + ch];
  const int64_t base = (((int64_t)b * 2 * H + 2 * y) * 2 * W + 2 * x) * C + ch;
  const int64_t rs = (int64_t)2 * W * C;
  return (dh[base] + dh[base + C]) + (dh[base + rs] + dh[base + rs + C]);
}

__global__ void prelu_bwd_kernel(const float* __restrict__ dh, const float* __restrict__ z,
                                 const float* __restrict__ slope, float* __restrict__ dz, float* __restrict__ dslope, int B,
                                 int H, int W, int C, int pool, unsigned* __restrict__ amax, double* __restrict__ ws,
                                 unsigned* __restrict__ ticket) {
  const float a = *slope;
  const int64_t n = (int64_t)B * H * W * C;
  double s = 0;
  float am = 0.f;
  for (int64_t i = blockIdx.x * (int64_t)blockDim.x + threadIdx.x; i < n; i += (int64_t)gridDim.x * blockDim.x) {
    const int ch = (int)(i % C);
    int64_t r = i / C;
    const int x = (int)(r % W);
    r /= W;
    const int y = (int)(r % H);
    const int b = (int)(r / H);
    const float g = load_dh(dh, b, y, x, ch, H, W, C, pool);
    const float v = z[i];
    if (v > 0.f) {
      dz[i] = g;
      am = fmaxf(am, fabsf(g));
    } else {
      dz[i] = a * g;
      am = fmaxf(am, fabsf(a * g));
      s += (double)g * (double)v;
    }
  }
  amax_commit(amax, am);
  s = block_sum(s);
  if (!dslope) return;
  if (threadIdx.x == 0) ws[blockIdx.x] = s;
  if (ordered_last_block(ticket)) {
    if (threadIdx.x == 0) *dslope += (float)ordered_sum(ws, gridDim.x, 1, 0);
    ordered_release(ticket);
  }
}
int k_prelu_bwd(fg_ctx* c, const float* dh, const float* z, const float* slope, float* dz, float* dslope, int B, int H,
                int W, int C, int pool) {
  const int64_t n = (int64_t)B * H * W * C;
  prelu_bwd_kernel<<<grid_for(n, 256, 132 * 8), 256, 0, c->stream>>>(dh, z, slope, dz, dslope, B, H, W, C, pool, take_amax(c),
                                                                    c->red_ws, c->red_ticket);
  LAUNCH_CHECK(c);
  return FG_OK;
}

__global__ void bn_stats_kernel(const float* __restrict__ z, double* __restrict__ acc, int64_t P, int C,
                                int64_t rows_per_block, double* __restrict__ ws, unsigned* __restrict__ ticket) {
  extern __shared__ double sm[];
  const int lanes = blockDim.x / C;
  const int ch = threadIdx.x % C, lane = threadIdx.x / C;
  const int64_t r0 = blockIdx.x * rows_per_block, r1 = min(P, r0 + rows_per_block);
  double s = 0, s2 = 0;
  for (int64_t r = r0 + lane; r < r1; r += lanes) {
    const double v = z[r * C + ch];
    s += v;
    s2 += v * v;
  }
  sm[threadIdx.x] = s;
  sm[blockDim.x + threadIdx.x] = s2;
  __syncthreads();
  if (lane == 0) {
    for (int l = 1; l < lanes; ++l) {
      s += sm[l * C + ch];
      s2 += sm[blockDim.x + l * C + ch];
    }
    ws[(int64_t)blockIdx.x * 2 * C + ch] = s;
    ws[(int64_t)blockIdx.x * 2 * C + C + ch] = s2;
  }
  if (ordered_last_block(ticket)) {
    for (int i = threadIdx.x; i < 2 * C; i += blockDim.x) acc[i] += ordered_sum(ws, gridDim.x, 2 * C, i);
    ordered_release(ticket);
  }
}
static inline int bn_block(int C) {
  int lanes = 256 / C;
  if (lanes < 1) lanes = 1;
  return C * lanes;
}
int k_bn_stats(fg_ctx* c, const float* z, double* acc, int64_t P, int C) {
  if (k_bn4_ok(C)) return k_bn_stats4(c, z, acc, P, C);
  if (C > 1024) {
    fg_set_error("BatchNorm with C=%d > 1024 unsupported", C);
    return FG_ERR_UNSUPPORTED;
  }
  FG_CUDA(cudaMemsetAsync(acc, 0, sizeof(double) * 2 * C, c->stream));
  const int block = bn_block(C);
  int grid = (int)std::min<int64_t>(c->sm_count * 4, (P + 63) / 64);
  if (grid < 1) grid = 1;
  const int64_t rpb = (P + grid - 1) / grid;
  FG_TRY(red_check(c, grid, 2 * C));
  bn_stats_kernel<<<grid, block, sizeof(double) * 2 * block, c->stream>>>(z, acc, P, C, rpb, c->red_ws, c->red_ticket);
  LAUNCH_CHECK(c);
  return FG_OK;
}
__global__ void bn_finalize_kernel(const double* __restrict__ acc, float* __restrict__ mean, float* __restrict__ istd,
                                   float* __restrict__ run_mean, float* __restrict__ run_var, int64_t P, int C) {
  const int ch = blockIdx.x * blockDim.x + threadIdx.x;
  if (ch >= C) return;
  const double n = (double)P;
  const double m = acc[ch] / n;
  double var = acc[C + ch] / n - m * m;
  if (var < 0) var = 0;
  mean[ch] = (float)m;
  istd[ch] = (float)(1.0 / sqrt(var + 1e-5));
  if (run_mean) run_mean[ch] = 0.9f * run_mean[ch] + 0.1f * (float)m;
  if (run_var) run_var[ch] = 0.9f * run_var[ch] + 0.1f * (float)(P > 1 ? var * n / (n - 1.0) : var);
}
int k_bn_finalize(fg_ctx* c, double* acc, float* mean, float* istd, float* run_mean, float* run_var, int64_t P, int C) {
  bn_finalize_kernel<<<(C + 127) / 128, 128, 0, c->stream>>>(acc, mean, istd, run_mean, run_var, P, C);
  LAUNCH_CHECK(c);
  return FG_OK;
}
constexpr int kBnSlices = 32;
__global__ void __launch_bounds__(256) bn_finalize_parts_kernel(const float* __restrict__ part, int nparts, double* __restrict__ slice_acc,
                                                                unsigned int* __restrict__ ticket, float* __restrict__ mean,
                                                                float* __restrict__ istd, float* __restrict__ run_mean,
                                                                float* __restrict__ run_var, int64_t P, int C) {
  __shared__ double sm[2][8][32];
  __shared__ bool last;
  const int lane = threadIdx.x & 31, g = threadIdx.x >> 5;
  const int ch = blockIdx.x * 32 + lane;
  const int per = (nparts + kBnSlices - 1) / kBnSlices;
  const int i0 = blockIdx.y * per, i1 = min(nparts, i0 + per);
  double s = 0, q = 0;
  if (ch < C)
    for (int i = i0 + g; i < i1; i += 8) {
      s += (double)part[((int64_t)i * 2 + 0) * C + ch];
      q += (double)part[((int64_t)i * 2 + 1) * C + ch];
    }
  sm[0][g][lane] = s;
  sm[1][g][lane] = q;
  __syncthreads();
  if (g == 0 && ch < C) {
    for (int k = 1; k < 8; ++k) {
      s += sm[0][k][lane];
      q += sm[1][k][lane];
    }
    slice_acc[((int64_t)blockIdx.y * 2 + 0) * C + ch] = s;
    slice_acc[((int64_t)blockIdx.y * 2 + 1) * C + ch] = q;
  }
  __threadfence();
  __syncthreads();
  if (threadIdx.x == 0) last = atomicAdd(ticket + blockIdx.x, 1u) == (unsigned)kBnSlices - 1;
  __syncthreads();
  if (!last) return;
  __threadfence();
  if (threadIdx.x == 0) ticket[blockIdx.x] = 0;
  if (g != 0 || ch >= C) return;
  s = 0;
  q = 0;
  for (int k = 0; k < kBnSlices; ++k) {
    s += slice_acc[((int64_t)k * 2 + 0) * C + ch];
    q += slice_acc[((int64_t)k * 2 + 1) * C + ch];
  }
  const double n = (double)P;
  const double m = s / n;
  double var = q / n - m * m;
  if (var < 0) var = 0;
  mean[ch] = (float)m;
  istd[ch] = (float)(1.0 / sqrt(var + 1e-5));
  if (run_mean) run_mean[ch] = 0.9f * run_mean[ch] + 0.1f * (float)m;
  if (run_var) run_var[ch] = 0.9f * run_var[ch] + 0.1f * (float)(P > 1 ? var * n / (n - 1.0) : var);
}
int k_bn_finalize_parts(fg_ctx* c, const float* part, int nparts, float* mean, float* istd, float* run_mean, float* run_var,
                        int64_t P, int C) {
  double* acc = c->bn_slice_acc;
  unsigned int* ticket = reinterpret_cast<unsigned int*>(acc + (size_t)kBnSlices * 2 * 256);
  bn_finalize_parts_kernel<<<dim3((C + 31) / 32, kBnSlices), 256, 0, c->stream>>>(part, nparts, acc, ticket, mean, istd, run_mean,
                                                                                run_var, P, C);
  LAUNCH_CHECK(c);
  return FG_OK;
}
__global__ void bn_eval_prep_kernel(const float* __restrict__ rm, const float* __restrict__ rv, float* __restrict__ mean,
                                    float* __restrict__ istd, int C) {
  const int ch = blockIdx.x * blockDim.x + threadIdx.x;
  if (ch >= C) return;
  mean[ch] = rm[ch];
  istd[ch] = 1.0f / sqrtf(rv[ch] + 1e-5f);
}
int k_bn_eval_prep(fg_ctx* c, const float* rm, const float* rv, float* mean, float* istd, int C) {
  bn_eval_prep_kernel<<<(C + 127) / 128, 128, 0, c->stream>>>(rm, rv, mean, istd, C);
  LAUNCH_CHECK(c);
  return FG_OK;
}
__global__ void bn_prelu_apply_kernel(const float* __restrict__ z, const float* __restrict__ mean,
                                      const float* __restrict__ istd, const float* __restrict__ gamma,
                                      const float* __restrict__ beta, const float* __restrict__ slope,
                                      float* __restrict__ h, float* __restrict__ hi, float* __restrict__ lo, int64_t n4,
                                      int C, unsigned* __restrict__ amax) {
  float am = 0.f;
  const bool act = slope != nullptr;
  const float a = act ? *slope : 1.f;
  const float4* z4 = reinterpret_cast<const float4*>(z);
  float4* h4 = reinterpret_cast<float4*>(h);
  float4* hi4 = reinterpret_cast<float4*>(hi);
  float4* lo4 = reinterpret_cast<float4*>(lo);
  for (int64_t i = blockIdx.x * (int64_t)blockDim.x + threadIdx.x; i < n4; i += (int64_t)gridDim.x * blockDim.x) {
    const int ch = (int)((i * 4) % C);
    const float4 v = z4[i];
    const float4 m = *reinterpret_cast<const float4*>(mean + ch);
    const float4 s = *reinterpret_cast<const float4*>(istd + ch);
    const float4 g = make_float4(gamma[ch], gamma[ch + 1], gamma[ch + 2], gamma[ch + 3]);
    const float4 b = make_float4(beta[ch], beta[ch + 1], beta[ch + 2], beta[ch + 3]);
    float4 o;
    o.x = g.x * ((v.x - m.x) * s.x) + b.x;
    o.y = g.y * ((v.y - m.y) * s.y) + b.y;
    o.z = g.z * ((v.z - m.z) * s.z) + b.z;
    o.w = g.w * ((v.w - m.w) * s.w) + b.w;
    if (act) {
      o.x = o.x > 0.f ? o.x : a * o.x;
      o.y = o.y > 0.f ? o.y : a * o.y;
      o.z = o.z > 0.f ? o.z : a * o.z;
      o.w = o.w > 0.f ? o.w : a * o.w;
    }
    if (h) h4[i] = o;
    am = amax4(am, o.x, o.y, o.z, o.w);
    if (hi) {
      float4 vh, vl;
      vh.x = __uint_as_float((__float_as_uint(o.x) + 0x1000u) & 0xFFFFE000u);
      vh.y = __uint_as_float((__float_as_uint(o.y) + 0x1000u) & 0xFFFFE000u);
      vh.z = __uint_as_float((__float_as_uint(o.z) + 0x1000u) & 0xFFFFE000u);
      vh.w = __uint_as_float((__float_as_uint(o.w) + 0x1000u) & 0xFFFFE000u);
      vl = make_float4(o.x - vh.x, o.y - vh.y, o.z - vh.z, o.w - vh.w);
      hi4[i] = vh;
      lo4[i] = vl;
    }
  }
  amax_commit(amax, am);
}
__global__ void bn_prelu_apply_scalar_kernel(const float* __restrict__ z, const float* __restrict__ mean,
                                             const float* __restrict__ istd, const float* __restrict__ gamma,
                                             const float* __restrict__ beta, const float* __restrict__ slope,
                                             float* __restrict__ h, int64_t n, int C) {
  const bool act = slope != nullptr;
  const float a = act ? *slope : 1.f;
  for (int64_t i = blockIdx.x * (int64_t)blockDim.x + threadIdx.x; i < n; i += (int64_t)gridDim.x * blockDim.x) {
    const int ch = (int)(i % C);
    float o = gamma[ch] * ((z[i] - mean[ch]) * istd[ch]) + beta[ch];
    if (act) o = o > 0.f ? o : a * o;
    h[i] = o;
  }
}
int k_bn_prelu_apply(fg_ctx* c, const float* z, const float* mean, const float* istd, const float* gamma,
                     const float* beta, const float* slope, float* h, int64_t P, int C, float* hi, float* lo) {
  const int64_t n = P * C;
  if (C % 4 == 0) {
    bn_prelu_apply_kernel<<<grid_for(n / 4, 256), 256, 0, c->stream>>>(z, mean, istd, gamma, beta, slope, h, hi, lo, n / 4, C,
                                                                       take_amax(c));
  } else {
    if (hi || !h) {
      fg_set_error("bn_prelu_apply: hi/lo outputs need C %% 4 == 0");
      return FG_ERR_UNSUPPORTED;
    }
    bn_prelu_apply_scalar_kernel<<<grid_for(n, 256), 256, 0, c->stream>>>(z, mean, istd, gamma, beta, slope, h, n, C);
  }
  LAUNCH_CHECK(c);
  return FG_OK;
}

__global__ void bn_prelu_bwd_reduce_kernel(const float* __restrict__ dh, const float* __restrict__ z,
                                           const float* __restrict__ mean, const float* __restrict__ istd,
                                           const float* __restrict__ gamma, const float* __restrict__ beta,
                                           const float* __restrict__ slope, double* __restrict__ acc,
                                           float* __restrict__ dslope, int B, int H, int W, int C, int pool,
                                           int64_t rows_per_block, double* __restrict__ ws, unsigned* __restrict__ ticket) {
  extern __shared__ double sm[];
  const int lanes = blockDim.x / C;
  const int ch = threadIdx.x % C, lane = threadIdx.x / C;
  const int64_t P = (int64_t)B * H * W;
  const int64_t r0 = blockIdx.x * rows_per_block, r1 = min(P, r0 + rows_per_block);
  const bool act = slope != nullptr;
  const float a = act ? *slope : 1.f;
  const float m = mean[ch], is = istd[ch], ga = gamma[ch], be = beta[ch];
  double sg = 0, sgx = 0, ss = 0;
  for (int64_t r = r0 + lane; r < r1; r += lanes) {
    float d;
    if (pool) {
      const uint32_t ru = (uint32_t)r;
      const int x = (int)(ru % (uint32_t)W);
      const uint32_t q = ru / (uint32_t)W;
      d = load_dh(dh, (int)(q / (uint32_t)H), (int)(q % (uint32_t)H), x, ch, H, W, C, 1);
    } else {
      d = dh[r * C + ch];
    }
    const float xh = (z[r * C + ch] - m) * is;
    float g = d;
    if (act) {
      const float u = ga * xh + be;
      if (!(u > 0.f)) {
        g = a * d;
        ss += (double)d * (double)u;
      }
    }
    sg += g;
    sgx += (double)g * (double)xh;
  }
  sm[threadIdx.x] = sg;
  sm[blockDim.x + threadIdx.x] = sgx;
  __syncthreads();
  if (lane == 0) {
    for (int l = 1; l < lanes; ++l) {
      sg += sm[l * C + ch];
      sgx += sm[blockDim.x + l * C + ch];
    }
    ws[(int64_t)blockIdx.x * (2 * C + 1) + ch] = sg;
    ws[(int64_t)blockIdx.x * (2 * C + 1) + C + ch] = sgx;
  }
  if (act) ss = block_sum(ss);
  if (threadIdx.x == 0) ws[(int64_t)blockIdx.x * (2 * C + 1) + 2 * C] = ss;
  if (ordered_last_block(ticket)) {
    for (int i = threadIdx.x; i < 2 * C; i += blockDim.x) acc[i] += ordered_sum(ws, gridDim.x, 2 * C + 1, i);
    if (act && dslope && threadIdx.x == 0) *dslope += (float)ordered_sum(ws, gridDim.x, 2 * C + 1, 2 * C);
    ordered_release(ticket);
  }
}
int k_bn_prelu_bwd_reduce(fg_ctx* c, const float* dh, const float* z, const float* mean, const float* istd,
                          const float* gamma, const float* beta, const float* slope, double* acc, float* dslope, int B,
                          int H, int W, int C, int pool) {
  if (!pool && k_bn4_ok(C))
    return k_bn_bwd_reduce4(c, dh, z, mean, istd, gamma, beta, slope, acc, dslope, (int64_t)B * H * W, C);
  if (C > 1024) return FG_ERR_UNSUPPORTED;
  FG_CUDA(cudaMemsetAsync(acc, 0, sizeof(double) * 2 * C, c->stream));
  const int64_t P = (int64_t)B * H * W;
  const int block = bn_block(C);
  int grid = (int)std::min<int64_t>(c->sm_count * 4, (P + 63) / 64);
  if (grid < 1) grid = 1;
  const int64_t rpb = (P + grid - 1) / grid;
  FG_TRY(red_check(c, grid, 2 * C + 1));
  bn_prelu_bwd_reduce_kernel<<<grid, block, sizeof(double) * 2 * block, c->stream>>>(dh, z, mean, istd, gamma, beta, slope,
                                                                                  acc, dslope, B, H, W, C, pool, rpb, c->red_ws,
                                                                                  c->red_ticket);
  LAUNCH_CHECK(c);
  return FG_OK;
}
__global__ void bn_bwd_finalize_kernel(const double* __restrict__ acc, float* __restrict__ mg, float* __restrict__ dgamma,
                                       float* __restrict__ dbeta, int64_t P, int C) {
  const int ch = blockIdx.x * blockDim.x + threadIdx.x;
  if (ch >= C) return;
  mg[ch] = (float)(acc[ch] / (double)P);
  mg[C + ch] = (float)(acc[C + ch] / (double)P);
  if (dgamma) dgamma[ch] += (float)acc[C + ch];
  if (dbeta) dbeta[ch] += (float)acc[ch];
}
int k_bn_bwd_finalize(fg_ctx* c, double* acc, float* mg, float* dgamma, float* dbeta, int64_t P, int C) {
  bn_bwd_finalize_kernel<<<(C + 127) / 128, 128, 0, c->stream>>>(acc, mg, dgamma, dbeta, P, C);
  LAUNCH_CHECK(c);
  return FG_OK;
}
__global__ void bn_prelu_bwd_apply_kernel(const float* __restrict__ dh, const float* __restrict__ z,
                                          const float* __restrict__ mean, const float* __restrict__ istd,
                                          const float* __restrict__ gamma, const float* __restrict__ beta,
                                          const float* __restrict__ slope, const float* __restrict__ mg,
                                          float* __restrict__ dz, int B, int H, int W, int C, int pool) {
  const bool act = slope != nullptr;
  const float a = act ? *slope : 1.f;
  const int64_t n = (int64_t)B * H * W * C;
  for (int64_t i = blockIdx.x * (int64_t)blockDim.x + threadIdx.x; i < n; i += (int64_t)gridDim.x * blockDim.x) {
    const int ch = (int)(i % C);
    int64_t r = i / C;
    const int x = (int)(r % W);
    r /= W;
    const int y = (int)(r % H);
    const int b = (int)(r / H);
    const float d = load_dh(dh, b, y, x, ch, H, W, C, pool);
    const float is = istd[ch], ga = gamma[ch];
    const float xh = (z[i] - mean[ch]) * is;
    float g = d;
    if (act) {
      const float u = ga * xh + beta[ch];
      if (!(u > 0.f)) g = a * d;
    }
    dz[i] = ga * is * (g - mg[ch] - xh * mg[C + ch]);
  }
}
__device__ void block_colsum_rows(const float (&bs)[4], int C, int n, double* ws, unsigned* ticket, float* dst,
                                  float* extra_dst, double extra = 0.0) {
  __shared__ float tb[256][4];
#pragma unroll
  for (int j = 0; j < 4; ++j) tb[threadIdx.x][j] = bs[j];
  __syncthreads();
  const int C4 = C / 4;
  double* row = ws + (int64_t)blockIdx.x * n;
  for (int i = threadIdx.x; i < C; i += blockDim.x) {
    double s = 0;
    for (int t = i / 4; t < (int)blockDim.x; t += C4) s += tb[t][i & 3];
    row[i] = s;
  }
  if (n > C && threadIdx.x == 0) row[C] = extra;
  if (ordered_last_block(ticket)) {
    if (dst)
      for (int i = threadIdx.x; i < C; i += blockDim.x) dst[i] += (float)ordered_sum(ws, gridDim.x, n, i);
    if (extra_dst && threadIdx.x == 0) *extra_dst += (float)ordered_sum(ws, gridDim.x, n, C);
    ordered_release(ticket);
  }
}

__global__ void bn_prelu_bwd_apply4_kernel(const float* __restrict__ dh, const float* __restrict__ z,
                                           const float* __restrict__ mean, const float* __restrict__ istd,
                                           const float* __restrict__ gamma, const float* __restrict__ beta,
                                           const float* __restrict__ slope, const float* __restrict__ mg,
                                           float* __restrict__ dz, float* __restrict__ hi, float* __restrict__ lo,
                                           float* __restrict__ dbias, int64_t n4, int C, unsigned* __restrict__ amax,
                                           double* __restrict__ ws, unsigned* __restrict__ ticket) {
  float am = 0.f;
  float bs[4] = {0.f, 0.f, 0.f, 0.f};
  const bool act = slope != nullptr;
  const float a = act ? *slope : 1.f;
  const float4* dh4 = reinterpret_cast<const float4*>(dh);
  const float4* z4 = reinterpret_cast<const float4*>(z);
  float4* dz4 = reinterpret_cast<float4*>(dz);
  float4* hi4 = reinterpret_cast<float4*>(hi);
  float4* lo4 = reinterpret_cast<float4*>(lo);
  const int C4 = C / 4;
  for (int64_t i = blockIdx.x * (int64_t)blockDim.x + threadIdx.x; i < n4; i += (int64_t)gridDim.x * blockDim.x) {
    const int ch = (int)(i % C4) * 4;
    const float4 d = dh4[i], v = z4[i];
    const float dv[4] = {d.x, d.y, d.z, d.w}, zv[4] = {v.x, v.y, v.z, v.w};
    float o[4];
#pragma unroll
    for (int j = 0; j < 4; ++j) {
      const float is = istd[ch + j], ga = gamma[ch + j];
      const float xh = (zv[j] - mean[ch + j]) * is;
      float g = dv[j];
      if (act) {
        const float u = ga * xh + beta[ch + j];
        if (!(u > 0.f)) g = a * g;
      }
      o[j] = ga * is * (g - mg[ch + j] - xh * mg[C + ch + j]);
    }
    dz4[i] = make_float4(o[0], o[1], o[2], o[3]);
    am = amax4(am, o[0], o[1], o[2], o[3]);
    bs[0] += o[0]; bs[1] += o[1]; bs[2] += o[2]; bs[3] += o[3];
    if (hi) {
      float h[4];
#pragma unroll
      for (int j = 0; j < 4; ++j) h[j] = __uint_as_float((__float_as_uint(o[j]) + 0x1000u) & 0xFFFFE000u);
      hi4[i] = make_float4(h[0], h[1], h[2], h[3]);
      lo4[i] = make_float4(o[0] - h[0], o[1] - h[1], o[2] - h[2], o[3] - h[3]);
    }
  }
  amax_commit(amax, am);
  if (dbias) block_colsum_rows(bs, C, C, ws, ticket, dbias, nullptr);
}
int k_bn_prelu_bwd_apply(fg_ctx* c, const float* dh, const float* z, const float* mean, const float* istd,
                         const float* gamma, const float* beta, const float* slope, const float* mg, float* dz, int B,
                         int H, int W, int C, int pool, float* hi, float* lo, float* dbias) {
  const int64_t n = (int64_t)B * H * W * C;
  if (!pool && C % 4 == 0 && C <= 1024 && 256 % (C / 4) == 0) {
    const int grid = grid_for(n / 4, 256);
    FG_TRY(red_check(c, grid, C));
    bn_prelu_bwd_apply4_kernel<<<grid, 256, 0, c->stream>>>(dh, z, mean, istd, gamma, beta, slope, mg, dz, hi, lo, dbias, n / 4,
                                                           C, take_amax(c), c->red_ws, c->red_ticket);
    LAUNCH_CHECK(c);
    return FG_OK;
  }
  if (hi) {
    fg_set_error("bn_prelu_bwd_apply: hi/lo outputs need the un-pooled float4 path");
    return FG_ERR_UNSUPPORTED;
  }
  bn_prelu_bwd_apply_kernel<<<grid_for(n, 256), 256, 0, c->stream>>>(dh, z, mean, istd, gamma, beta, slope, mg, dz, B, H,
                                                                    W, C, pool);
  LAUNCH_CHECK(c);
  if (dbias) return k_colsum_add(c, dz, dbias, (int64_t)B * H * W, C, 0, 0);
  return FG_OK;
}

__device__ __forceinline__ float sigmoidf_(float x) { return 1.0f / (1.0f + expf(-x)); }
__global__ void sigmoid_fwd_kernel(const float* __restrict__ z, float* __restrict__ y, int64_t n) {
  for (int64_t i = blockIdx.x * (int64_t)blockDim.x + threadIdx.x; i < n; i += (int64_t)gridDim.x * blockDim.x)
    y[i] = sigmoidf_(z[i]);
}
int k_sigmoid_fwd(fg_ctx* c, const float* z, float* y, int64_t n) {
  sigmoid_fwd_kernel<<<grid_for(n, 256), 256, 0, c->stream>>>(z, y, n);
  LAUNCH_CHECK(c);
  return FG_OK;
}
__global__ void sigmoid_bwd_kernel(const float* __restrict__ dy, const float* __restrict__ y, float* __restrict__ dz,
                                   int64_t n) {
  for (int64_t i = blockIdx.x * (int64_t)blockDim.x + threadIdx.x; i < n; i += (int64_t)gridDim.x * blockDim.x) {
    const float v = y[i];
    dz[i] = dy[i] * v * (1.0f - v);
  }
}
int k_sigmoid_bwd(fg_ctx* c, const float* dy, const float* y, float* dz, int64_t n) {
  sigmoid_bwd_kernel<<<grid_for(n, 256), 256, 0, c->stream>>>(dy, y, dz, n);
  LAUNCH_CHECK(c);
  return FG_OK;
}
int k_sigmoid_grad_mul(fg_ctx* c, const float* dout, const float* out, float* dlogit, int n) {
  return k_sigmoid_bwd(c, dout, out, dlogit, n);
}

__device__ __forceinline__ uint64_t splitmix64(uint64_t x) {
  x += 0x9E3779B97F4A7C15ull;
  x = (x ^ (x >> 30)) * 0xBF58476D1CE4E5B9ull;
  x = (x ^ (x >> 27)) * 0x94D049BB133111EBull;
  return x ^ (x >> 31);
}
__global__ void masks_generate_kernel(float* __restrict__ masks, int B, uint64_t seed, float p_spatial, float p_drop,
                                      const uint64_t* __restrict__ seed_dev) {
  if (seed_dev) seed += *seed_dev * 2;
  const int64_t n = (int64_t)B * kMaskPerSample;
  for (int64_t i = blockIdx.x * (int64_t)blockDim.x + threadIdx.x; i < n; i += (int64_t)gridDim.x * blockDim.x) {
    const int j = (int)(i % kMaskPerSample);
    const uint64_t r = splitmix64(seed * 0x100000001B3ull + (uint64_t)i);
    const float u = (float)(r >> 40) * (1.0f / 16777216.0f);
    masks[i] = u >= (j < 960 ? p_spatial : p_drop) ? 1.f : 0.f;
  }
}
__global__ void set_u64_kernel(uint64_t* dst, uint64_t v) { *dst = v; }
int k_set_u64(fg_ctx* c, uint64_t* dst, uint64_t v) {
  set_u64_kernel<<<1, 1, 0, c->stream>>>(dst, v);
  LAUNCH_CHECK(c);
  return FG_OK;
}
int k_masks_generate(fg_ctx* c, float* masks, int B, uint64_t seed, float p_spatial, float p_drop, const uint64_t* seed_dev) {
  masks_generate_kernel<<<grid_for((int64_t)B * kMaskPerSample, 256), 256, 0, c->stream>>>(masks, B, seed, p_spatial,
                                                                                          p_drop, seed_dev);
  LAUNCH_CHECK(c);
  return FG_OK;
}

__device__ __forceinline__ float4 prelu4(float4 v, float a) {
  v.x = v.x > 0.f ? v.x : a * v.x;
  v.y = v.y > 0.f ? v.y : a * v.y;
  v.z = v.z > 0.f ? v.z : a * v.z;
  v.w = v.w > 0.f ? v.w : a * v.w;
  return v;
}
__device__ __forceinline__ void split4(const float4& o, float4* hi, float4* lo, uint32_t i) {
  float4 h;
  h.x = __uint_as_float((__float_as_uint(o.x) + 0x1000u) & 0xFFFFE000u);
  h.y = __uint_as_float((__float_as_uint(o.y) + 0x1000u) & 0xFFFFE000u);
  h.z = __uint_as_float((__float_as_uint(o.z) + 0x1000u) & 0xFFFFE000u);
  h.w = __uint_as_float((__float_as_uint(o.w) + 0x1000u) & 0xFFFFE000u);
  hi[i] = h;
  lo[i] = make_float4(o.x - h.x, o.y - h.y, o.z - h.z, o.w - h.w);
}
__global__ void d_act_pool_fwd_kernel(const float* __restrict__ z, const float* __restrict__ slope,
                                      const float* __restrict__ masks, int moff, float eval_scale, float* __restrict__ p,
                                      float4* __restrict__ hi, float4* __restrict__ lo, int B, int H, int W, int C,
                                      unsigned* __restrict__ amax) {
  float am = 0.f;
  const float a = *slope;
  const uint32_t Ho = H / 2, Wo = W / 2, C4 = C / 4;
  const uint32_t n = (uint32_t)B * Ho * Wo * C4;
  const float4* z4 = reinterpret_cast<const float4*>(z);
  float4* p4 = reinterpret_cast<float4*>(p);
  for (uint32_t i = blockIdx.x * blockDim.x + threadIdx.x; i < n; i += gridDim.x * blockDim.x) {
    const uint32_t c4 = i % C4;
    uint32_t r = i / C4;
    const uint32_t xo = r % Wo;
    r /= Wo;
    const uint32_t yo = r % Ho, b = r / Ho;
    float4 m = make_float4(eval_scale, eval_scale, eval_scale, eval_scale);
    if (masks) m = *reinterpret_cast<const float4*>(masks + (size_t)b * kMaskPerSample + moff + c4 * 4);
    const uint32_t base = ((b * H + 2 * yo) * W + 2 * xo) * C4 + c4, rs = (uint32_t)W * C4;
    const float4 v0 = prelu4(z4[base], a), v1 = prelu4(z4[base + C4], a), v2 = prelu4(z4[base + rs], a),
                 v3 = prelu4(z4[base + rs + C4], a);
    float4 o;
    o.x = (v0.x * m.x + v1.x * m.x + v2.x * m.x + v3.x * m.x) * 0.25f;
    o.y = (v0.y * m.y + v1.y * m.y + v2.y * m.y + v3.y * m.y) * 0.25f;
    o.z = (v0.z * m.z + v1.z * m.z + v2.z * m.z + v3.z * m.z) * 0.25f;
    o.w = (v0.w * m.w + v1.w * m.w + v2.w * m.w + v3.w * m.w) * 0.25f;
    p4[i] = o;
    am = amax4(am, o.x, o.y, o.z, o.w);
    if (hi) split4(o, hi, lo, i);
  }
  amax_commit(amax, am);
}
int k_d_act_pool_fwd(fg_ctx* c, const float* z, const float* slope, const float* masks, int moff, float eval_scale,
                     float* p, int B, int H, int W, int C, float* hi, float* lo) {
  const int64_t n = (int64_t)B * (H / 2) * (W / 2) * C / 4;
  if (C % 4 || (moff % 4) || (int64_t)B * H * W * C >= ((int64_t)1 << 31)) {
    fg_set_error("d_act_pool_fwd: unsupported shape (C %% 4, size)");
    return FG_ERR_UNSUPPORTED;
  }
  d_act_pool_fwd_kernel<<<grid_for(n, 256), 256, 0, c->stream>>>(z, slope, masks, moff, eval_scale, p, reinterpret_cast<float4*>(hi),
                                                                 reinterpret_cast<float4*>(lo), B, H, W, C, take_amax(c));
  LAUNCH_CHECK(c);
  return FG_OK;
}
__global__ void d_act_pool_bwd_kernel(const float* __restrict__ dp, const float* __restrict__ z,
                                      const float* __restrict__ slope, const float* __restrict__ masks, int moff,
                                      float eval_scale, float* __restrict__ dz, float* __restrict__ dslope,
                                      float4* __restrict__ hi, float4* __restrict__ lo, float* __restrict__ dbias, int B,
                                      int H, int W, int C, unsigned* __restrict__ amax, double* __restrict__ ws,
                                      unsigned* __restrict__ ticket) {
  float am = 0.f;
  float bs[4] = {0.f, 0.f, 0.f, 0.f};
  const float a = *slope;
  const uint32_t Ho = H / 2, Wo = W / 2, C4 = C / 4;
  const uint32_t n = (uint32_t)B * Ho * Wo * C4;
  const float4* z4 = reinterpret_cast<const float4*>(z);
  const float4* dp4 = reinterpret_cast<const float4*>(dp);
  float4* dz4 = reinterpret_cast<float4*>(dz);
  float s = 0.f;
  double sd = 0;
  for (uint32_t i = blockIdx.x * blockDim.x + threadIdx.x; i < n; i += gridDim.x * blockDim.x) {
    const uint32_t c4 = i % C4;
    uint32_t r = i / C4;
    const uint32_t xo = r % Wo;
    r /= Wo;
    const uint32_t yo = r % Ho, b = r / Ho;
    float4 m = make_float4(eval_scale, eval_scale, eval_scale, eval_scale);
    if (masks) m = *reinterpret_cast<const float4*>(masks + (size_t)b * kMaskPerSample + moff + c4 * 4);
    const float4 d = dp4[i];
    const float4 g = make_float4(d.x * 0.25f * m.x, d.y * 0.25f * m.y, d.z * 0.25f * m.z, d.w * 0.25f * m.w);
    const uint32_t base = ((b * H + 2 * yo) * W + 2 * xo) * C4 + c4, rs = (uint32_t)W * C4;
    s = 0.f;
#pragma unroll
    for (int q = 0; q < 4; ++q) {
      const uint32_t idx = base + (q & 1) * C4 + (q >> 1) * rs;
      const float4 v = z4[idx];
      float4 o;
      o.x = v.x > 0.f ? g.x : a * g.x;
      o.y = v.y > 0.f ? g.y : a * g.y;
      o.z = v.z > 0.f ? g.z : a * g.z;
      o.w = v.w > 0.f ? g.w : a * g.w;
      if (!(v.x > 0.f)) s = fmaf(g.x, v.x, s);
      if (!(v.y > 0.f)) s = fmaf(g.y, v.y, s);
      if (!(v.z > 0.f)) s = fmaf(g.z, v.z, s);
      if (!(v.w > 0.f)) s = fmaf(g.w, v.w, s);
      dz4[idx] = o;
      am = amax4(am, o.x, o.y, o.z, o.w);
      bs[0] += o.x; bs[1] += o.y; bs[2] += o.z; bs[3] += o.w;
      if (hi) split4(o, hi, lo, idx);
    }
    sd += (double)s;
  }
  amax_commit(amax, am);
  sd = block_sum(sd);
  if (dbias || dslope) block_colsum_rows(bs, dbias ? (int)C : 0, (dbias ? (int)C : 0) + 1, ws, ticket, dbias, dslope, sd);
}
int k_d_act_pool_bwd(fg_ctx* c, const float* dp, const float* z, const float* slope, const float* masks, int moff,
                     float eval_scale, float* dz, float* dslope, int B, int H, int W, int C, float* hi, float* lo,
                     float* dbias) {
  const int64_t n = (int64_t)B * (H / 2) * (W / 2) * C / 4;
  if (C % 4 || (moff % 4) || (int64_t)B * H * W * C >= ((int64_t)1 << 31)) {
    fg_set_error("d_act_pool_bwd: unsupported shape (C %% 4, size)");
    return FG_ERR_UNSUPPORTED;
  }
  const bool fuse = dbias && C <= 512 && 256 % (C / 4) == 0;
  const int grid = grid_for(n, 256, 132 * 8);
  FG_TRY(red_check(c, grid, C + 1));
  d_act_pool_bwd_kernel<<<grid, 256, 0, c->stream>>>(dp, z, slope, masks, moff, eval_scale, dz, dslope,
                                                    reinterpret_cast<float4*>(hi), reinterpret_cast<float4*>(lo),
                                                    fuse ? dbias : nullptr, B, H, W, C, take_amax(c), c->red_ws, c->red_ticket);
  LAUNCH_CHECK(c);
  if (dbias && !fuse) return k_colsum_add(c, dz, dbias, (int64_t)B * H * W, C, 0, 0);
  return FG_OK;
}
__global__ void lin_act_drop_fwd_kernel(const float* __restrict__ z, const float* __restrict__ slope,
                                        const float* __restrict__ masks, int moff, float scale, float* __restrict__ h,
                                        int B, int N, unsigned* __restrict__ amax) {
  float am = 0.f;
  const float a = *slope;
  const int64_t n = (int64_t)B * N;
  for (int64_t i = blockIdx.x * (int64_t)blockDim.x + threadIdx.x; i < n; i += (int64_t)gridDim.x * blockDim.x) {
    const int j = (int)(i % N);
    const int b = (int)(i / N);
    const float v = z[i];
    const float act = v > 0.f ? v : a * v;
    const float o = masks ? act * masks[(int64_t)b * kMaskPerSample + moff + j] * scale : act;
    h[i] = o;
    am = fmaxf(am, fabsf(o));
  }
  amax_commit(amax, am);
}
int k_lin_act_drop_fwd(fg_ctx* c, const float* z, const float* slope, const float* masks, int moff, float scale,
                       float* h, int B, int N) {
  lin_act_drop_fwd_kernel<<<grid_for((int64_t)B * N, 256), 256, 0, c->stream>>>(z, slope, masks, moff, scale, h, B, N, take_amax(c));
  LAUNCH_CHECK(c);
  return FG_OK;
}
__global__ void lin_act_drop_bwd_kernel(const float* __restrict__ dh, const float* __restrict__ z,
                                        const float* __restrict__ slope, const float* __restrict__ masks, int moff,
                                        float scale, float* __restrict__ dz, float* __restrict__ dslope, int B, int N,
                                        unsigned* __restrict__ amax, double* __restrict__ ws, unsigned* __restrict__ ticket) {
  float am = 0.f;
  const float a = *slope;
  const int64_t n = (int64_t)B * N;
  double s = 0;
  for (int64_t i = blockIdx.x * (int64_t)blockDim.x + threadIdx.x; i < n; i += (int64_t)gridDim.x * blockDim.x) {
    const int j = (int)(i % N);
    const int b = (int)(i / N);
    const float g = masks ? dh[i] * masks[(int64_t)b * kMaskPerSample + moff + j] * scale : dh[i];
    const float v = z[i];
    if (v > 0.f) {
      dz[i] = g;
      am = fmaxf(am, fabsf(g));
    } else {
      dz[i] = a * g;
      am = fmaxf(am, fabsf(a * g));
      s += (double)g * (double)v;
    }
  }
  amax_commit(amax, am);
  s = block_sum(s);
  if (!dslope) return;
  if (threadIdx.x == 0) ws[blockIdx.x] = s;
  if (ordered_last_block(ticket)) {
    if (threadIdx.x == 0) *dslope += (float)ordered_sum(ws, gridDim.x, 1, 0);
    ordered_release(ticket);
  }
}
int k_lin_act_drop_bwd(fg_ctx* c, const float* dh, const float* z, const float* slope, const float* masks, int moff,
                       float scale, float* dz, float* dslope, int B, int N) {
  lin_act_drop_bwd_kernel<<<grid_for((int64_t)B * N, 256, 132), 256, 0, c->stream>>>(dh, z, slope, masks, moff, scale, dz,
                                                                                   dslope, B, N, take_amax(c), c->red_ws,
                                                                                   c->red_ticket);
  LAUNCH_CHECK(c);
  return FG_OK;
}

__device__ __forceinline__ float bce_term(float x, float t) {
  const float eps = 1e-12f;
  return t * logf(x + eps) + (1.0f - t) * logf(1.0f - x + eps);
}
__device__ __forceinline__ float bce_grad(float x, float t, float invN) {
  const float eps = 1e-12f;
  return -(t - x) / (x * (1.0f - x + eps) + eps) * invN;
}
__global__ void sigmoid_bce_kernel(const float* __restrict__ logit, float* __restrict__ out, float* __restrict__ dlogit,
                                   float* __restrict__ loss_out, float* __restrict__ tail4, int B, int n_ones) {
  double s = 0;
  int c0 = 0, c1 = 0, c2 = 0, c3 = 0;
  const float invN = 1.0f / (float)B;
  for (int i = threadIdx.x; i < B; i += blockDim.x) {
    const float y = sigmoidf_(logit[i]);
    const float t = i < n_ones ? 1.f : 0.f;
    out[i] = y;
    s += (double)bce_term(y, t);
    dlogit[i] = bce_grad(y, t, invN) * y * (1.0f - y);
    const bool pred1 = y > 0.5f;
    if (t > 0.5f) {
      if (pred1) c0++; else c1++;
    } else {
      if (pred1) c2++; else c3++;
    }
  }
  s = block_sum(s);
  const double d0 = block_sum((double)c0), d1 = block_sum((double)c1), d2 = block_sum((double)c2),
               d3 = block_sum((double)c3);
  if (threadIdx.x == 0) {
    *loss_out = (float)(-s / (double)B);
    if (tail4) {
      tail4[0] = (float)d0;
      tail4[1] = (float)d1;
      tail4[2] = (float)d2;
      tail4[3] = (float)d3;
    }
  }
}
int k_sigmoid_bce(fg_ctx* c, const float* logit, float* out, float* dlogit, float* loss_out, float* tail4, int B,
                  int n_ones) {
  sigmoid_bce_kernel<<<1, 256, 0, c->stream>>>(logit, out, dlogit, loss_out, tail4, B, n_ones);
  LAUNCH_CHECK(c);
  return FG_OK;
}
__global__ void bce_fwd_kernel(const float* __restrict__ x, const float* __restrict__ t, int n, float* __restrict__ loss) {
  double s = 0;
  for (int i = threadIdx.x; i < n; i += blockDim.x) s += (double)bce_term(x[i], t[i]);
  s = block_sum(s);
  if (threadIdx.x == 0) *loss = (float)(-s / (double)n);
}
__global__ void bce_bwd_kernel(const float* __restrict__ x, const float* __restrict__ t, int n, float* __restrict__ dx) {
  const float invN = 1.0f / (float)n;
  for (int i = blockIdx.x * blockDim.x + threadIdx.x; i < n; i += gridDim.x * blockDim.x) dx[i] = bce_grad(x[i], t[i], invN);
}
int k_bce_fwd(fg_ctx* c, const float* x, const float* t, int n, float* loss_out) {
  bce_fwd_kernel<<<1, 256, 0, c->stream>>>(x, t, n, loss_out);
  LAUNCH_CHECK(c);
  return FG_OK;
}
int k_bce_bwd(fg_ctx* c, const float* x, const float* t, int n, float* dx) {
  bce_bwd_kernel<<<grid_for(n, 256), 256, 0, c->stream>>>(x, t, n, dx);
  LAUNCH_CHECK(c);
  return FG_OK;
}

__global__ void penalty_loss_kernel(const float* __restrict__ p, int64_t n, float l1, float l2, float* __restrict__ loss,
                                    double* __restrict__ ws, unsigned* __restrict__ ticket) {
  double s1 = 0, s2 = 0;
  for (int64_t i = blockIdx.x * (int64_t)blockDim.x + threadIdx.x; i < n; i += (int64_t)gridDim.x * blockDim.x) {
    const double v = p[i];
    s1 += fabs(v);
    s2 += v * v;
  }
  s1 = block_sum(s1);
  s2 = block_sum(s2);
  if (threadIdx.x == 0) ws[blockIdx.x] = l1 * s1 + l2 * s2 * 0.5;
  if (ordered_last_block(ticket)) {
    if (threadIdx.x == 0) *loss += (float)ordered_sum(ws, gridDim.x, 1, 0);
    ordered_release(ticket);
  }
}
int k_penalty_loss(fg_ctx* c, const float* p, int64_t n, float l1, float l2, float* loss_inout) {
  penalty_loss_kernel<<<grid_for(n, 256, kOptRedRows), 256, 0, c->stream>>>(p, n, l1, l2, loss_inout, c->red_ws_opt,
                                                                           c->red_ticket + 1);
  LAUNCH_CHECK(c);
  return FG_OK;
}
__device__ __forceinline__ float step_size(const fg_hyper& h, int opt, float lr, double t) {
  if (opt != FG_OPT_ADAM) return lr;
  return (float)((double)lr * sqrt(1.0 - pow((double)h.beta2, t)) / (1.0 - pow((double)h.beta1, t)));
}
__global__ void gate_prep_kernel(DeviceStats* st, float* acc_hist, int net, fg_hyper h, const float* tail4, float total, int opt) {
  if (threadIdx.x != 0 || blockIdx.x != 0) return;
  if (net == FG_NET_D) {
    int interval = h.accs_interval;
    if (interval < 1) interval = 1;
    if (interval > kAccHistMax) interval = kAccHistMax;
    const float correct = tail4[0] + tail4[3];
    const float tV = correct / total;
    for (int i = 0; i < 4; ++i) st->conf[i] = (int)(tail4[i] + 0.5f);
    st->acc_D = tV;
    acc_hist[st->acc_head] = tV;
    st->acc_head = (st->acc_head + 1) % interval;
    if (st->acc_count < interval) st->acc_count++;
    double m = 0;
    for (int i = 0; i < st->acc_count; ++i) m += acc_hist[i];
    m /= st->acc_count;
    const int go = m < (double)h.D_maxAcc ? 1 : 0;
    st->do_train_D = go;
    st->trained_D = go;
    if (go) {
      st->t_D += 1;
      st->step_D = step_size(h, opt, h.lr_D, (double)st->t_D);
    }
  } else {
    st->do_train_G = 1;
    st->t_G += 1;
    st->step_G = step_size(h, opt, h.lr_G, (double)st->t_G);
  }
}
int k_gate_and_prep(fg_ctx* c, DeviceStats* st, float* acc_hist, int net, const fg_hyper* h, const float* tail4, int B,
                    float world) {
  gate_prep_kernel<<<1, 32, 0, c->stream>>>(st, acc_hist, net, *h, tail4, (float)B * world, net == FG_NET_D ? c->opt_D : c->opt_G);
  LAUNCH_CHECK(c);
  return FG_OK;
}
__global__ void adam_kernel(float* __restrict__ p, float* __restrict__ g, float* __restrict__ m, float* __restrict__ v,
                            int64_t n, float beta1, float beta2, float eps, float l1_grad, float l2, float clampv,
                            float grad_scale, const float* __restrict__ step_dev, const int* __restrict__ flag_dev,
                            float step_host, int update, int mode, float mom, const int* __restrict__ t_dev) {
  if (flag_dev && *flag_dev == 0) update = 0;
  const float step = step_dev ? *step_dev : step_host;
  const bool first = t_dev ? *t_dev == 1 : false;
  const bool pen = (l1_grad != 0.f) || (l2 != 0.f);
  for (int64_t i = blockIdx.x * (int64_t)blockDim.x + threadIdx.x; i < n; i += (int64_t)gridDim.x * blockDim.x) {
    const float pv = p[i];
    float gv = g[i] * grad_scale;
    if (pen) {
      const float sg = pv > 0.f ? 1.f : (pv < 0.f ? -1.f : 0.f);
      gv += sg * l1_grad + pv * l2;
    }
    if (clampv != 0.f) gv = fminf(fmaxf(gv, -clampv), clampv);
    g[i] = gv;
    if (!update) continue;
    if (mode == FG_OPT_ADAM) {
      const float mv = m[i] * beta1 + (1.0f - beta1) * gv;
      const float vv = v[i] * beta2 + (1.0f - beta2) * gv * gv;
      m[i] = mv;
      v[i] = vv;
      p[i] = pv - step * mv / (sqrtf(vv) + eps);
    } else if (mode == FG_OPT_ADAGRAD) {
      const float vv = v[i] + gv * gv;
      v[i] = vv;
      p[i] = pv - step * gv / (sqrtf(vv) + 1e-10f);
    } else {
      float ge = gv;
      if (mom != 0.f) {
        ge = first ? gv : m[i] * mom + (1.0f - mom) * gv;
        m[i] = ge;
      }
      p[i] = pv - step * ge;
    }
  }
}
__global__ void gemv_fwd_kernel(const float* __restrict__ x, const float* __restrict__ w, const float* __restrict__ bias,
                                float* __restrict__ out, int B, int K) {
  const int row = (blockIdx.x * blockDim.x + threadIdx.x) >> 5, lane = threadIdx.x & 31;
  if (row >= B) return;
  float s = 0.f;
  for (int k = lane; k < K; k += 32) s = fmaf(x[(size_t)row * K + k], w[k], s);
#pragma unroll
  for (int o = 16; o > 0; o >>= 1) s += __shfl_xor_sync(0xffffffffu, s, o);
  if (lane == 0) out[row] = s + (bias ? bias[0] : 0.f);
}
__global__ void gemv_dgrad_kernel(const float* __restrict__ dy, const float* __restrict__ w, float* __restrict__ dx, int B,
                                  int K) {
  const int n = B * K;
  for (int i = blockIdx.x * blockDim.x + threadIdx.x; i < n; i += gridDim.x * blockDim.x) dx[i] = dy[i / K] * w[i % K];
}
__global__ void gemv_wgrad_kernel(const float* __restrict__ x, const float* __restrict__ dy, float* __restrict__ dw,
                                  float* __restrict__ db, int B, int K) {
  const int k = blockIdx.x * blockDim.x + threadIdx.x;
  if (k < K) {
    float s = 0.f;
    for (int b = 0; b < B; ++b) s = fmaf(dy[b], x[(size_t)b * K + k], s);
    dw[k] += s;
  }
  if (k == 0 && db) {
    float s = 0.f;
    for (int b = 0; b < B; ++b) s += dy[b];
    db[0] += s;
  }
}
int k_gemv_fwd(fg_ctx* c, const float* x, const float* w, const float* bias, float* out, int B, int K) {
  gemv_fwd_kernel<<<(B * 32 + 255) / 256, 256, 0, c->stream>>>(x, w, bias, out, B, K);
  LAUNCH_CHECK(c);
  return FG_OK;
}
int k_gemv_dgrad(fg_ctx* c, const float* dy, const float* w, float* dx, int B, int K) {
  gemv_dgrad_kernel<<<grid_for((int64_t)B * K, 256), 256, 0, c->stream>>>(dy, w, dx, B, K);
  LAUNCH_CHECK(c);
  return FG_OK;
}
int k_gemv_wgrad_add(fg_ctx* c, const float* x, const float* dy, float* dw, float* db, int B, int K) {
  gemv_wgrad_kernel<<<(K + 127) / 128, 128, 0, c->stream>>>(x, dy, dw, db, B, K);
  LAUNCH_CHECK(c);
  return FG_OK;
}

int k_adam(fg_ctx* c, float* p, const float* g, float* m, float* v, int64_t n, float beta1, float beta2, float eps,
           float l1_grad, float l2, float clampv, float grad_scale, const float* step_dev, const int* flag_dev,
           float step_host, float* g_out) {
  (void)g_out;
  adam_kernel<<<grid_for(n, 256, 132 * 8), 256, 0, c->stream>>>(p, const_cast<float*>(g), m, v, n, beta1, beta2, eps,
                                                               l1_grad, l2, clampv, grad_scale, step_dev, flag_dev,
                                                               step_host, 1, FG_OPT_ADAM, 0.f, nullptr);
  LAUNCH_CHECK(c);
  return FG_OK;
}
int k_optim_update(fg_ctx* c, int mode, float* p, float* g, float* m, float* v, int64_t n, float beta1, float beta2, float eps,
                   float mom, float l1_grad, float l2, float clampv, float grad_scale, const float* step_dev,
                   const int* flag_dev, const int* t_dev) {
  adam_kernel<<<grid_for(n, 256, 132 * 8), 256, 0, c->stream>>>(p, g, m, v, n, beta1, beta2, eps, l1_grad, l2, clampv, grad_scale,
                                                               step_dev, flag_dev, 0.f, 1, mode, mom, t_dev);
  LAUNCH_CHECK(c);
  return FG_OK;
}
```

face_generator_b200/csrc/nets.cu:

```cuda
#include <algorithm>

#include "convl.h"
#include "fg_internal.h"
#include "k_conv_tc.h"

DLayout make_d_layout(int C) {
  DLayout L;
  const int cin[4] = {C, 64, 128, 256}, cout[4] = {64, 128, 256, 512};
  int64_t o = 0;
  for (int i = 0; i < 4; ++i) {
    L.cW[i] = o; o += (int64_t)cout[i] * cin[i] * 9;
    L.cb[i] = o; o += cout[i];
    L.ca[i] = o; o += 1;
  }
  L.L1W = o; o += 512 * 2048;
  L.L1b = o; o += 512;
  L.a5 = o; o += 1;
  L.L2W = o; o += 512 * 512;
  L.L2b = o; o += 512;
  L.a6 = o; o += 1;
  L.L3W = o; o += 512;
  L.L3b = o; o += 1;
  L.total = o;
  return L;
}

namespace {
const int kDcin[4] = {0 , 64, 128, 256}, kDcout[4] = {64, 128, 256, 512}, kDhw[4] = {32, 16, 8, 4};
const int kDmoff[4] = {0, 64, 192, 448};
inline int dcin(const fg_ctx* c, int i) { return i == 0 ? c->C : kDcin[i]; }

int dalloc(fg_ctx* c, float** p, size_t n) { return fg_dalloc(c, c->allocs, p, n); }
}

int net_alloc(fg_ctx* c) {
  const size_t B = c->maxB, C = c->C;
  c->dl = make_d_layout(c->C);
  NetPair& p = c->net;
  FG_TRY(pair_alloc(c, c->allocs, p, make_g_layout(c->C, 32).total, c->dl.total, true));
  p.optim_timer[0] = "hbm.optim.G";
  p.optim_timer[1] = "hbm.optim.D";
  c->ownPG = p.PG; c->ownPD = p.PD; c->ownGG = p.gG; c->ownGD = p.gD;
  FG_TRY(dalloc(c, &c->tail_sep, 2 * kGradTail));
  float* tmp = nullptr;
  FG_TRY(dalloc(c, &c->lop_sx, 2));
  FG_TRY(dalloc(c, &c->lop_sy, 2));
  {
    float* sd = nullptr;
    FG_TRY(dalloc(c, &sd, 2));
    c->seed_dev = reinterpret_cast<uint64_t*>(sd);
  }
  c->wgrad_ws_elems = std::max<size_t>(9 * 512 * 256, 8192 * (128 + kNoiseDim));
  FG_TRY(dalloc(c, &c->wgrad_ws, c->wgrad_ws_elems));
  c->splitk_ws_elems = (size_t)c->sm_count * 4 * 128 * 128;
  FG_TRY(dalloc(c, &c->splitk_ws, c->splitk_ws_elems));
  c->red_ws_elems = (size_t)4 << 20;
  FG_TRY(dalloc(c, reinterpret_cast<float**>(&c->red_ws), 2 * c->red_ws_elems));
  FG_TRY(dalloc(c, reinterpret_cast<float**>(&c->red_ws_opt), 2 * kOptRedRows));
  FG_TRY(dalloc(c, reinterpret_cast<float**>(&c->red_ticket), 2));
  FG_TRY(dalloc(c, reinterpret_cast<float**>(&c->bwd_claim), 1));
  FG_TRY(dalloc(c, &c->small_ws, (size_t)kSmallMaxParts * 9 * 4 * 128));
  FG_TRY(dalloc(c, &tmp, 4 * 256 * 2));
  c->bn_acc = (double*)tmp;
  FG_TRY(dalloc(c, &tmp, 32 * 2 * 256 * 2 + 64));
  c->bn_slice_acc = (double*)tmp;
  FG_TRY(dalloc(c, &c->bn_parts, B * 2048));
  FG_TRY(dalloc(c, &c->D_x, B * 1024 * C));
  for (int i = 0; i < 4; ++i) {
    const size_t n = B * (size_t)kDhw[i] * kDhw[i] * kDcout[i];
    FG_TRY(dalloc(c, &c->D_z[i], n));
    FG_TRY(dalloc(c, &c->D_p[i], n / 4));
  }
  FG_TRY(dalloc(c, &c->D_zl1, B * 512));
  FG_TRY(dalloc(c, &c->D_hl1, B * 512));
  FG_TRY(dalloc(c, &c->D_zl2, B * 512));
  FG_TRY(dalloc(c, &c->D_hl2, B * 512));
  FG_TRY(dalloc(c, &c->D_logit, B));
  FG_TRY(dalloc(c, &c->D_out, B));
  FG_TRY(dalloc(c, &c->D_masks, B * kMaskPerSample));
  FG_TRY(dalloc(c, &c->D_dlogit, B));
  FG_TRY(dalloc(c, &c->D_dh, B * 512));
  FG_TRY(dalloc(c, &c->D_dzl, B * 512));
  FG_TRY(dalloc(c, &c->D_dz, B * 65536));
  FG_TRY(dalloc(c, &c->D_dp, B * 16384));
  FG_TRY(dalloc(c, &c->D_dx, B * 1024 * C));
  FG_TRY(dalloc(c, &c->D_targets, B));
  c->io_dev_elems = std::max<size_t>(B * 1024 * C, B * kMaskPerSample);
  FG_TRY(dalloc(c, &c->io_dev, c->io_dev_elems));
  FG_TRY(dalloc(c, &c->io_dev2, c->io_dev_elems));
  {
    ConvLEnv& e = c->env;
    e.c = c;
    e.maxB = c->maxB;
    e.allocs = &c->allocs;
    e.ws = c->wgrad_ws;
    FG_TRY(dalloc(c, &e.dy.hi, B * 131072));
    FG_TRY(dalloc(c, &e.dy.lo, B * 131072));
    static const GenDesc g32{32, "", 128, true};
    FG_TRY(gen_alloc(e, c->G, g32));
    ScalePairs& sp = c->D_pairs;
    FG_TRY(sp.alloc(c, c->allocs, 1 + 2 * 6));
    FG_TRY(sp.take(&e.dy.s));
    const DLayout& dl = c->dl;
    auto conv = [&](ConvL& L, int Cin, int Cout, int k, int H, int64_t w_off, int64_t b_off, const char* tf, const char* td,
                    const char* tw) {
      L.Cin = Cin; L.Cout = Cout; L.k = k; L.H = H;
      L.w_off = w_off; L.b_off = b_off;
      L.tf = tf; L.td = td; L.tw = tw;
    };
    static const char* tf[4] = {"D.C1.fwd", "D.C2.fwd", "D.C3.fwd", "D.C4.fwd"};
    static const char* td[4] = {"D.C1.dgrad", "D.C2.dgrad", "D.C3.dgrad", "D.C4.dgrad"};
    static const char* tw[4] = {"D.C1.wgrad", "D.C2.wgrad", "D.C3.wgrad", "D.C4.wgrad"};
    for (int i = 0; i < 4; ++i) conv(c->Dc[i], dcin(c, i), kDcout[i], 3, kDhw[i], dl.cW[i], dl.cb[i], tf[i], td[i], tw[i]);
    conv(c->DL1, 2048, 512, 1, 1, dl.L1W, dl.L1b, "D.L1.fwd", "D.L1.dgrad", "D.L1.wgrad");
    c->DL1.cA = 512; c->DL1.cS = 4;
    conv(c->DL2, 512, 512, 1, 1, dl.L2W, dl.L2b, "D.L2.fwd", "D.L2.dgrad", "D.L2.wgrad");
    for (ConvL* L : {&c->Dc[0], &c->Dc[1], &c->Dc[2], &c->Dc[3], &c->DL1, &c->DL2}) {
      FG_TRY(sp.take(&L->x.s));
      FG_TRY(sp.take(&L->sdy));
      FG_TRY(convl_alloc(e, *L));
    }
  }
  FG_TRY(dalloc(c, &c->in_real, B * 1024 * C));
  FG_TRY(dalloc(c, &c->in_noiseD, B * kNoiseDim));
  FG_TRY(dalloc(c, &c->in_noiseG, B * kNoiseDim));
  FG_TRY(dalloc(c, &c->in_masksD, B * kMaskPerSample));
  FG_TRY(dalloc(c, &c->in_masksG, B * kMaskPerSample));
  FG_CUDA(cudaStreamSynchronize(c->stream));
  return FG_OK;
}

void net_free(fg_ctx* c) {
  pair_free(c->net);
  for (void* p : c->allocs) cudaFree(p);
  c->allocs.clear();
  if (c->stage_pinned) cudaFreeHost(c->stage_pinned);
  for (int i = 0; i < 8; ++i)
    if (c->scratch[i]) cudaFree(c->scratch[i]);
}

int net_pack_D(fg_ctx* c) {
  if (c->net.D_packed) return FG_OK;
  for (int i = 0; i < 4; ++i) FG_TRY(convl_pack(c, c->Dc[i], c->net.PD));
  FG_TRY(convl_pack(c, c->DL1, c->net.PD));
  FG_TRY(convl_pack(c, c->DL2, c->net.PD));
  c->net.D_packed = true;
  return FG_OK;
}

int net_D_forward(fg_ctx* c, const float* x, int B, bool training, const fg_hyper* h) {
  FG_REQUIRE(B >= 1 && B <= c->maxB, "D forward: batch %d out of range [1,%d]", B, c->maxB);
  FG_TRY(net_pack_D(c));
  FG_TRY(c->D_pairs.reset(c));
  const DLayout& L = c->dl;
  float* P = c->net.PD;
  if (x != c->D_x)
    FG_CUDA(cudaMemcpyAsync(c->D_x, x, sizeof(float) * (size_t)B * 1024 * c->C, cudaMemcpyDeviceToDevice, c->stream));
  c->D_B = B;
  c->D_train = training;
  const float* masks = training ? c->D_masks : nullptr;
  const float* cur = c->D_x;
  for (int i = 0; i < 4; ++i) {
    const int H = kDhw[i];
    FG_TRY(convl_fwd(c->env, c->Dc[i], cur, P, c->D_z[i], B));
    TcOp& nx = (i < 3 ? c->Dc[i + 1] : c->DL1).x;
    nx.split_ready = convl_tc_fwd(c, i < 3 ? c->Dc[i + 1] : c->DL1) && !tc_f16(c);
    {
      AmaxInto am(c, nx);
      FG_TRY(k_d_act_pool_fwd(c, c->D_z[i], P + L.ca[i], masks, kDmoff[i], 1.0f - h->p_spatial, c->D_p[i], B, H, H,
                              kDcout[i], nx.split_ready ? nx.hi : nullptr, nx.split_ready ? nx.lo : nullptr));
    }
    cur = c->D_p[i];
  }
  const float scale = 1.0f / (1.0f - h->p_drop);
  c->D_drop_scale = scale;
  c->D_spatial_eval = 1.0f - h->p_spatial;
  FG_TRY(convl_fwd(c->env, c->DL1, c->D_p[3], P, c->D_zl1, B));
  {
    AmaxInto am(c, c->DL2.x);
    FG_TRY(k_lin_act_drop_fwd(c, c->D_zl1, P + L.a5, masks, 960, scale, c->D_hl1, B, 512));
  }
  FG_TRY(convl_fwd(c->env, c->DL2, c->D_hl1, P, c->D_zl2, B));
  FG_TRY(k_lin_act_drop_fwd(c, c->D_zl2, P + L.a6, masks, 1472, scale, c->D_hl2, B, 512));
  {
    ScopedTimer tm(c, "D.L3.fwd");
    FG_TRY(k_gemv_fwd(c, c->D_hl2, P + L.L3W, P + L.L3b, c->D_logit, B, 512));
  }
  c->D_fwd_valid = true;
  return FG_OK;
}

int net_D_backward(fg_ctx* c, const float* dlogit, bool want_wgrad, bool want_dx) {
  if (!c->D_fwd_valid) {
    fg_set_error("D backward needs a preceding D forward");
    return FG_ERR_STATE;
  }
  const DLayout& L = c->dl;
  float *P = c->net.PD, *G = c->net.gD;
  const int B = c->D_B;
  const float* masks = c->D_train ? c->D_masks : nullptr;
  const float scale = c->D_drop_scale, eval_scale = c->D_spatial_eval;
  FG_TRY(c->D_pairs.reset(c));
  if (want_wgrad) {
    ScopedTimer tm(c, "D.L3.wgrad");
    FG_TRY(k_gemv_wgrad_add(c, c->D_hl2, dlogit, G + L.L3W, G + L.L3b, B, 512));
  }
  {
    ScopedTimer tm(c, "D.L3.dgrad");
    FG_TRY(k_gemv_dgrad(c, dlogit, P + L.L3W, c->D_dh, B, 512));
  }
  TcOp& dy = c->env.dy;
  float* GD = want_wgrad ? G : nullptr;
  {
    AmaxInto am(c, c->DL2.sdy, &dy.amax_ready);
    FG_TRY(k_lin_act_drop_bwd(c, c->D_dh, c->D_zl2, P + L.a6, masks, 1472, scale, c->D_dzl, want_wgrad ? G + L.a6 : nullptr, B,
                              512));
  }
  FG_TRY(convl_bwd(c->env, c->DL2, c->D_hl1, c->D_dzl, GD, c->D_dh, B));
  {
    AmaxInto am(c, c->DL1.sdy, &dy.amax_ready);
    FG_TRY(k_lin_act_drop_bwd(c, c->D_dh, c->D_zl1, P + L.a5, masks, 960, scale, c->D_dzl, want_wgrad ? G + L.a5 : nullptr, B,
                              512));
  }
  FG_TRY(convl_bwd(c->env, c->DL1, c->D_p[3], c->D_dzl, GD, c->D_dp, B));
  for (int i = 3; i >= 0; --i) {
    const int H = kDhw[i];
    dy.split_ready = convl_tc_bwd(c, c->Dc[i]) && !tc_f16(c);
    dy.bias_ready = want_wgrad;
    {
      AmaxInto am(c, c->Dc[i].sdy, &dy.amax_ready);
      FG_TRY(k_d_act_pool_bwd(c, c->D_dp, c->D_z[i], P + L.ca[i], masks, kDmoff[i], eval_scale, c->D_dz,
                              want_wgrad ? G + L.ca[i] : nullptr, B, H, H, kDcout[i], dy.split_ready ? dy.hi : nullptr,
                              dy.split_ready ? dy.lo : nullptr, want_wgrad ? G + L.cb[i] : nullptr));
    }
    float* din = i > 0 ? c->D_dp : want_dx ? c->D_dx : nullptr;
    FG_TRY(convl_bwd(c->env, c->Dc[i], i == 0 ? c->D_x : c->D_p[i - 1], c->D_dz, GD, din, B));
  }
  return FG_OK;
}

static int train_step_body(fg_ctx* c, const fg_hyper* h, int B, const float* real, const float* noiseD, const float* noiseG,
                           const float* masksD, const float* masksG) {
  const uint64_t seed = 0;
  const uint64_t* seed_dev = c->seed_dev;
  const int Bh = B / 2, C = c->C;
  const size_t img = (size_t)C * 1024;
  const float world = (float)c->world;
  FG_TRY(gen_forward(c->env, c->G, c->net, noiseD, Bh, true));
  FG_TRY(k_nchw_to_nhwc(c, real, c->D_x, Bh, C, 1024));
  FG_CUDA(cudaMemcpyAsync(c->D_x + Bh * img, c->G.y, sizeof(float) * Bh * img, cudaMemcpyDeviceToDevice, c->stream));
  if (masksD)
    FG_CUDA(cudaMemcpyAsync(c->D_masks, masksD, sizeof(float) * (size_t)B * kMaskPerSample, cudaMemcpyDeviceToDevice,
                            c->stream));
  else
    FG_TRY(k_masks_generate(c, c->D_masks, B, seed * 2 + 1, h->p_spatial, h->p_drop, seed_dev));
  FG_TRY(pair_zero_grads(c, c->net, FG_NET_D));
  FG_TRY(net_D_forward(c, c->D_x, B, true, h));
  FG_TRY(k_sigmoid_bce(c, c->D_logit, c->D_out, c->D_dlogit, &c->net.dstats->loss_D, c->net.tailD, B, Bh));
  if (c->debug_keep) {
    const float* src[8] = {c->D_z[0], c->D_z[1], c->D_z[2], c->D_z[3], c->D_zl1, c->D_zl2, c->D_logit, c->D_out};
    const size_t per[8] = {65536, 32768, 16384, 8192, 512, 512, 1, 1};
    for (int i = 0; i < 8; ++i) {
      if (!c->keep_D[i]) FG_TRY(dalloc(c, &c->keep_D[i], (size_t)c->maxB * per[i]));
      FG_CUDA(cudaMemcpyAsync(c->keep_D[i], src[i], sizeof(float) * B * per[i], cudaMemcpyDeviceToDevice, c->stream));
    }
    c->keep_B = B;
  }
  FG_TRY(net_D_backward(c, c->D_dlogit, true, false));
  const bool overlap = c->world > 1 && c->dp_overlap && !c->timing;
  if (overlap) {
    if (!c->comm_stream) {
      FG_CUDA(cudaStreamCreateWithFlags(&c->comm_stream, cudaStreamNonBlocking));
      FG_CUDA(cudaEventCreateWithFlags(&c->ev_fork, cudaEventDisableTiming));
      FG_CUDA(cudaEventCreateWithFlags(&c->ev_join, cudaEventDisableTiming));
    }
    FG_CUDA(cudaEventRecord(c->ev_fork, c->stream));
    FG_CUDA(cudaStreamWaitEvent(c->comm_stream, c->ev_fork, 0));
    cudaStream_t compute = c->stream;
    c->stream = c->comm_stream;
    int r = pair_allreduce_grads(c, c->net, FG_NET_D);
    if (r == FG_OK) r = pair_gate(c, c->net, FG_NET_D, h, B, world);
    if (r == FG_OK) r = pair_optim(c, c->net, FG_NET_D, h, 1.0f / world);
    if (r == FG_OK && cudaEventRecord(c->ev_join, c->comm_stream) != cudaSuccess) r = FG_ERR_CUDA;
    c->stream = compute;
    FG_TRY(r);
  } else {
    FG_TRY(pair_allreduce_grads(c, c->net, FG_NET_D));
    FG_TRY(pair_gate(c, c->net, FG_NET_D, h, B, world));
    FG_TRY(pair_optim(c, c->net, FG_NET_D, h, 1.0f / world));
  }
  FG_TRY(pair_zero_grads(c, c->net, FG_NET_G));
  {
    static const int reserve = getenv("FG_DP_RESERVE_SMS") ? atoi(getenv("FG_DP_RESERVE_SMS")) : 0;
    c->reserve_sms = overlap ? reserve : 0;
    const int r = gen_forward(c->env, c->G, c->net, noiseG, B, true);
    c->reserve_sms = 0;
    FG_TRY(r);
  }
  if (overlap) FG_CUDA(cudaStreamWaitEvent(c->stream, c->ev_join, 0));
  if (masksG)
    FG_CUDA(cudaMemcpyAsync(c->D_masks, masksG, sizeof(float) * (size_t)B * kMaskPerSample, cudaMemcpyDeviceToDevice,
                            c->stream));
  else
    FG_TRY(k_masks_generate(c, c->D_masks, B, seed * 2 + 2, h->p_spatial, h->p_drop, seed_dev));
  FG_TRY(net_D_forward(c, c->G.y, B, true, h));
  FG_TRY(k_sigmoid_bce(c, c->D_logit, c->D_out, c->D_dlogit, &c->net.dstats->loss_G, c->net.tailG, B, B));
  FG_TRY(net_D_backward(c, c->D_dlogit, false, true));
  FG_TRY(gen_backward(c->env, c->G, c->net, c->D_dx, nullptr));
  FG_TRY(pair_allreduce_grads(c, c->net, FG_NET_G));
  FG_TRY(pair_gate(c, c->net, FG_NET_G, h, B, world));
  FG_TRY(pair_optim(c, c->net, FG_NET_G, h, 1.0f / world));
  FG_CUDA(cudaMemcpyAsync(c->net.hstats, c->net.dstats, sizeof(DeviceStats), cudaMemcpyDeviceToHost, c->stream));
  return FG_OK;
}

int net_train_step(fg_ctx* c, const fg_hyper* h, int B, const float* real, const float* noiseD, const float* noiseG,
                   const float* masksD, const float* masksG, uint64_t seed, bool allow_graph) {
  FG_REQUIRE(B >= 4 && B % 2 == 0 && B <= c->maxB, "train step: batch %d must be even, >=4 and <= %d", B, c->maxB);
  return net_graph_run(
      c, c->net, B, h, {real, noiseD, noiseG, masksD, masksG}, seed,
      [&]() { return train_step_body(c, h, B, real, noiseD, noiseG, masksD, masksG); }, allow_graph);
}
```

Measured before the change: 37610.

## Fuse generator BN+PReLU+final conv+sigmoid into edge conv kernels

The generator's last BatchNorm+PReLU apply is folded into the edge reduce-conv kernel as a prologue on the TMA-loaded tile, and sigmoid is applied in the epilogue. In backward, the BN/PReLU backward reduction is fused into the expand (dgrad) kernel using an ordered cross-block sum. The D-step forward also skips writing h2, since only the G step needs it for backward. This removes several full passes over the 128-channel activation. The cost is extra per-tile compute, a block-wide sync, and double-precision reductions inside the conv kernels.

Result: faster. 38570, median of 6 (+2.6%).

```diff
diff --git a/face_generator_b200/csrc/convl.cu b/face_generator_b200/csrc/convl.cu
--- a/face_generator_b200/csrc/convl.cu
+++ b/face_generator_b200/csrc/convl.cu
@@ -31,6 +31,12 @@
 }
 
 bool convl_tc_fwd(const fg_ctx* c, const ConvL& L) { return tc_f(c, L, 1); }
+bool convl_edge_fwd(const fg_ctx* c, const ConvL& L, int B) {
+  return !(L.pad_out && c->conv_impl != FG_CONV_SIMT) && !tc_f(c, L, B) && c->edge_impl && k_edge_eligible(L.geom(B));
+}
+bool convl_edge_dgrad(const fg_ctx* c, const ConvL& L, int B) {
+  return !tc_d(c, L, B) && c->edge_impl && k_edge_eligible(L.geom_d(B));
+}
 bool convl_tc_bwd(const fg_ctx* c, const ConvL& L) { return tc_f(c, L, 1) && tc_d(c, L, 1); }
 
 int tc_op_split(fg_ctx* c, TcOp& op, const float* x, int64_t n, bool f16) {
@@ -145,7 +151,7 @@
     return tc_conv_fwd(c, L.x.hi, L.x.lo, L.Wf_hi, L.Wf_lo, bias, out, gk, 0, nullptr, nullptr, h, os);
   }
   ScopedTimer t(c, L.tf);
-  if (c->edge_impl && k_edge_eligible(g)) return k_conv_edge(c, in, L.Wp, bias, out, g);
+  if (convl_edge_fwd(c, L, B)) return k_conv_edge(c, in, L.Wp, bias, out, g);
   return k_small_eligible(g) ? k_conv_small(c, in, L.Wp, bias, out, g) : k_conv_simt(c, in, L.Wp, bias, out, g);
 }
 
@@ -200,7 +206,7 @@
   if (din) {
     ScopedTimer t(c, L.td);
     if (d_tc) return tc_conv_fwd(c, e.dy.hi, e.dy.lo, L.Wd_hi, L.Wd_lo, nullptr, din, gd, 0, nullptr, nullptr, h, osy);
-    if (c->edge_impl && k_edge_eligible(gd)) return k_conv_edge(c, dy, L.Wpd, nullptr, din, gd);
+    if (convl_edge_dgrad(c, L, B)) return k_conv_edge(c, dy, L.Wpd, nullptr, din, gd);
     return k_small_eligible(gd) ? k_conv_small(c, dy, L.Wpd, nullptr, din, gd) : k_conv_simt(c, dy, L.Wpd, nullptr, din, gd);
   }
   return FG_OK;
diff --git a/face_generator_b200/csrc/convl.h b/face_generator_b200/csrc/convl.h
--- a/face_generator_b200/csrc/convl.h
+++ b/face_generator_b200/csrc/convl.h
@@ -24,6 +24,8 @@
 int convl_alloc(ConvLEnv& e, ConvL& L);
 bool convl_tc_fwd(const fg_ctx* c, const ConvL& L);
 bool convl_tc_bwd(const fg_ctx* c, const ConvL& L);
+bool convl_edge_fwd(const fg_ctx* c, const ConvL& L, int B);
+bool convl_edge_dgrad(const fg_ctx* c, const ConvL& L, int B);
 int convl_pack(fg_ctx* c, ConvL& L, const float* P);
 int convl_fwd(ConvLEnv& e, ConvL& L, const float* in, const float* P, float* out, int B);
 int convl_bwd(ConvLEnv& e, ConvL& L, const float* in, const float* dy, float* G, float* din, int B);
@@ -36,6 +38,6 @@
 
 int gen_alloc(ConvLEnv& e, UpsGen& G, const GenDesc& d);
 int gen_pack(fg_ctx* c, UpsGen& G, NetPair& p);
-int gen_forward(ConvLEnv& e, UpsGen& G, NetPair& p, const float* noise, int B, bool training);
+int gen_forward(ConvLEnv& e, UpsGen& G, NetPair& p, const float* noise, int B, bool training, bool keep_h2 = true);
 int gen_backward(ConvLEnv& e, UpsGen& G, NetPair& p, const float* dy, float* dnoise);
 void gen_debug_rows(const UpsGen& G, std::vector<DebugTensor>& rows);
diff --git a/face_generator_b200/csrc/fg_internal.h b/face_generator_b200/csrc/fg_internal.h
--- a/face_generator_b200/csrc/fg_internal.h
+++ b/face_generator_b200/csrc/fg_internal.h
@@ -176,6 +176,7 @@
   float *bn_mean[2] = {nullptr, nullptr}, *bn_istd[2] = {nullptr, nullptr}, *bn_mg = nullptr;
   int B = 0;
   bool train = true, valid = false;
+  bool h2_valid = false;
   int pack_key = -1;
   std::deque<std::string> names;
   const char *t_bn2_finalize = nullptr, *t_bn2_stats = nullptr, *t_bn2_apply = nullptr, *t_bn2_bwd_reduce = nullptr,
@@ -350,6 +351,11 @@
 
 bool k_edge_eligible(const ConvGeom& g);
 int k_conv_edge(fg_ctx* c, const float* in, const float* Wp, const float* bias, float* out, ConvGeom g);
+int k_gen_tail_fwd(fg_ctx* c, const float* z2, const float* mean, const float* istd, const float* gamma, const float* beta,
+                   const float* slope, const float* Wp, const float* bias, float* h, float* z3, float* y, ConvGeom g);
+int k_gen_tail_bwd_reduce(fg_ctx* c, const float* dz3, const float* Wpd, float* dh2, ConvGeom gd, const float* z2,
+                          const float* mean, const float* istd, const float* gamma, const float* beta, const float* slope,
+                          double* acc, float* dslope);
 
 inline int red_check(fg_ctx* c, int64_t rows, int64_t n) {
   if (rows * n > (int64_t)c->red_ws_elems) {
diff --git a/face_generator_b200/csrc/gen.cu b/face_generator_b200/csrc/gen.cu
--- a/face_generator_b200/csrc/gen.cu
+++ b/face_generator_b200/csrc/gen.cu
@@ -113,7 +113,7 @@
 }
 }
 
-int gen_forward(ConvLEnv& e, UpsGen& G, NetPair& p, const float* noise, int B, bool training) {
+int gen_forward(ConvLEnv& e, UpsGen& G, NetPair& p, const float* noise, int B, bool training, bool keep_h2) {
   fg_ctx* c = e.c;
   FG_REQUIRE(B >= 1 && B <= e.maxB, "G forward: batch %d out of range [1,%d]", B, e.maxB);
   FG_TRY(gen_pack(c, G, p));
@@ -144,19 +144,28 @@
   parts = training ? 1 : 0;
   FG_TRY(upsl_fwd(e, C2, G.h1, P, G.z2, B, &parts));
   FG_TRY(bn_stats(c, G, p, 1, G.z2, B, training, parts, G.t_bn2_finalize, G.t_bn2_stats));
-  {
-    ScopedTimer tm(c, G.t_bn2_apply);
-    FG_TRY(k_bn_prelu_apply(c, G.z2, G.bn_mean[1], G.bn_istd[1], P + L.g2, P + L.be2, P + L.a3, G.h2, (int64_t)B * S * S, 128));
-  }
-  FG_TRY(convl_fwd(e, G.GC3, G.h2, P, G.z3, B));
-  FG_TRY(k_sigmoid_fwd(c, G.z3, G.y, (int64_t)B * S * S * G.C));
+  ConvL& C3 = G.GC3;
+  const bool fused = convl_edge_fwd(c, C3, B);
+  if (fused) {
+    ScopedTimer tm(c, C3.tf);
+    FG_TRY(k_gen_tail_fwd(c, G.z2, G.bn_mean[1], G.bn_istd[1], P + L.g2, P + L.be2, P + L.a3, C3.Wp, P + C3.b_off,
+                          keep_h2 ? G.h2 : nullptr, G.z3, G.y, C3.geom(B)));
+  } else {
+    {
+      ScopedTimer tm(c, G.t_bn2_apply);
+      FG_TRY(k_bn_prelu_apply(c, G.z2, G.bn_mean[1], G.bn_istd[1], P + L.g2, P + L.be2, P + L.a3, G.h2, (int64_t)B * S * S, 128));
+    }
+    FG_TRY(convl_fwd(e, C3, G.h2, P, G.z3, B));
+    FG_TRY(k_sigmoid_fwd(c, G.z3, G.y, (int64_t)B * S * S * G.C));
+  }
   G.valid = true;
+  G.h2_valid = keep_h2 || !fused;
   return FG_OK;
 }
 
 int gen_backward(ConvLEnv& e, UpsGen& G, NetPair& p, const float* dy, float* dnoise) {
   fg_ctx* c = e.c;
-  if (!G.valid || !G.train) {
+  if (!G.valid || !G.train || !G.h2_valid) {
     fg_set_error("G backward needs a preceding training-mode G forward");
     return FG_ERR_STATE;
   }
@@ -166,8 +175,14 @@
   const int B = G.B, S = G.S, h = S / 2;
   FG_TRY(G.pairs.reset(c));
   FG_TRY(k_sigmoid_bwd(c, dy, G.y, G.dz3, (int64_t)B * S * S * G.C));
-  FG_TRY(convl_bwd(e, G.GC3, G.h2, G.dz3, g, G.dfull, B));
-  {
+  ConvL& C3 = G.GC3;
+  if (convl_edge_dgrad(c, C3, B)) {
+    FG_TRY(convl_bwd(e, C3, G.h2, G.dz3, g, nullptr, B));
+    ScopedTimer tm(c, C3.td);
+    FG_TRY(k_gen_tail_bwd_reduce(c, G.dz3, C3.Wpd, G.dfull, C3.geom_d(B), G.z2, G.bn_mean[1], G.bn_istd[1], P + L.g2, P + L.be2,
+                                 P + L.a3, c->bn_acc, g + L.a3));
+  } else {
+    FG_TRY(convl_bwd(e, C3, G.h2, G.dz3, g, G.dfull, B));
     ScopedTimer tm(c, G.t_bn2_bwd_reduce);
     FG_TRY(k_bn_prelu_bwd_reduce(c, G.dfull, G.z2, G.bn_mean[1], G.bn_istd[1], P + L.g2, P + L.be2, P + L.a3, c->bn_acc,
                                  g + L.a3, B, S, S, 128, 0));
@@ -212,5 +227,5 @@
                                {"G.y", G.y, n3, B}, {"G.dz2", G.dz2, n2, B}, {"G.dz1", G.dz1, n1, B}, {"G.dz0", G.dz0, n0, B},
                                {"G.bn_mean1", G.bn_mean[0], 256, 1}, {"G.bn_istd1", G.bn_istd[0], 256, 1},
                                {"G.bn_mean2", G.bn_mean[1], 128, 1}, {"G.bn_istd2", G.bn_istd[1], 128, 1}})
-    rows.push_back({r.name, G.valid ? r.p : nullptr, r.per, r.B});
-}
+    rows.push_back({r.name, G.valid && (r.p != G.h2 || G.h2_valid) ? r.p : nullptr, r.per, r.B});
+}
diff --git a/face_generator_b200/csrc/k_act.cuh b/face_generator_b200/csrc/k_act.cuh
--- /dev/null
+++ b/face_generator_b200/csrc/k_act.cuh
@@ -0,0 +1,17 @@
+#pragma once
+
+__device__ __forceinline__ float bn_prelu1(float z, float mean, float istd, float gamma, float beta, bool act, float slope) {
+  const float u = gamma * ((z - mean) * istd) + beta;
+  return act ? (u > 0.f ? u : slope * u) : u;
+}
+
+__device__ __forceinline__ float bn_prelu_bwd1(float z, float dh, float mean, float istd, float gamma, float beta, float slope,
+                                               float& xh, double& su) {
+  xh = (z - mean) * istd;
+  const float u = gamma * xh + beta;
+  if (u > 0.f) return dh;
+  su += (double)dh * (double)u;
+  return slope * dh;
+}
+
+__device__ __forceinline__ float sigmoidf_(float x) { return 1.0f / (1.0f + expf(-x)); }
diff --git a/face_generator_b200/csrc/k_conv_edge.cu b/face_generator_b200/csrc/k_conv_edge.cu
--- a/face_generator_b200/csrc/k_conv_edge.cu
+++ b/face_generator_b200/csrc/k_conv_edge.cu
@@ -3,7 +3,9 @@
 #include <algorithm>
 
 #include "fg_internal.h"
+#include "k_act.cuh"
 #include "k_conv_tc.h"
+#include "k_ordered.cuh"
 
 namespace {
 constexpr int kW = 32;
@@ -45,14 +47,24 @@
       : "memory");
 }
 
+__device__ __forceinline__ void sts128(uint32_t addr, float4 v) {
+  asm volatile("st.shared.v4.f32 [%0], {%1, %2, %3, %4};" ::"r"(addr), "f"(v.x), "f"(v.y), "f"(v.z), "f"(v.w) : "memory");
+}
+
 constexpr int kRedRows = 4;
 template <int VEC>
 constexpr uint32_t red_tile_bytes() { return (kRedRows + 2) * (kW + 2) * 32 * VEC * 4; }
 
-template <int NS, int VEC>
+struct BnTail {
+  const float *mean, *istd, *gamma, *beta, *slope;
+  float *h, *y;
+};
+
+template <int NS, int VEC, bool BNP>
 __global__ void __launch_bounds__(256, 1) conv_reduce_kernel(const __grid_constant__ CUtensorMap tmap, const float* __restrict__ Wp,
                                                              const float* __restrict__ bias, float* __restrict__ out, int H,
-                                                             int nunits) {
+                                                             int nunits, BnTail bt) {
+  static_assert(!BNP || VEC == 4, "the BatchNorm prologue maps 4 channels to a lane");
   constexpr int C = 32 * VEC;
   constexpr int PX = NS == 1 ? 16 : 4;
   constexpr uint32_t kTile = red_tile_bytes<VEC>();
@@ -83,6 +95,17 @@
       for (int j = 0; j < VEC; ++j) w[t][n][j] = Wp[(t * NS + n) * C + lane * VEC + j];
   float bv = 0.f;
   if (bias && (lane & 15) < PX * NS) bv = bias[(lane & 15) % NS];
+  float bm[4], bs[4], bg[4], bb[4], ba = 1.f;
+  if (BNP) {
+#pragma unroll
+    for (int j = 0; j < 4; ++j) {
+      bm[j] = bt.mean[lane * 4 + j];
+      bs[j] = bt.istd[lane * 4 + j];
+      bg[j] = bt.gamma[lane * 4 + j];
+      bb[j] = bt.beta[lane * 4 + j];
+    }
+    ba = *bt.slope;
+  }
   const int row = warp >> 1, xh = (warp & 1) * 16;
   int it = 0;
   for (int unit = blockIdx.x; unit < nunits; unit += gridDim.x, ++it) {
@@ -91,6 +114,26 @@
     mbar_wait(full + buf, (it >> 1) & 1);
     const uint32_t tile = smem_u32(smem + buf * kTile) + (uint32_t)lane * VEC * 4;
     const int b = unit / strips, y = (unit - b * strips) * kRedRows + row;
+    if (BNP) {
+      const int y0 = (unit - b * strips) * kRedRows - 1;
+      const uint32_t base = smem_u32(smem + buf * kTile);
+      for (int i = threadIdx.x; i < (kRedRows + 2) * (kW + 2) * 32; i += 256) {
+        const int p = i >> 5, r = p / (kW + 2), x = p - r * (kW + 2) - 1, gy = y0 + r;
+        float4 v = make_float4(0.f, 0.f, 0.f, 0.f);
+        if (gy >= 0 && gy < H && x >= 0 && x < kW) {
+          const float4 z = lds128(base + (uint32_t)i * 16);
+          v.x = bn_prelu1(z.x, bm[0], bs[0], bg[0], bb[0], true, ba);
+          v.y = bn_prelu1(z.y, bm[1], bs[1], bg[1], bb[1], true, ba);
+          v.z = bn_prelu1(z.z, bm[2], bs[2], bg[2], bb[2], true, ba);
+          v.w = bn_prelu1(z.w, bm[3], bs[3], bg[3], bb[3], true, ba);
+          if (bt.h && r >= 1 && r <= kRedRows)
+            *reinterpret_cast<float4*>(bt.h + ((size_t)(b * H + gy) * kW + x) * C + lane * 4) = v;
+        }
+        sts128(base + (uint32_t)i * 16, v);
+      }
+      asm volatile("fence.proxy.async.shared::cta;" ::: "memory");
+      __syncthreads();
+    }
 #pragma unroll 1
     for (int g = 0; g < 16 / PX; ++g) {
       const int x0 = xh + g * PX;
@@ -138,17 +181,30 @@
         }
       }
       const float tot = r[0] + __shfl_xor_sync(0xffffffffu, r[0], 16);
-      if (lane < PX * NS) out[((size_t)(b * H + y) * kW + x0) * NS + lane] = tot + bv;
+      if (lane < PX * NS) {
+        const size_t o = ((size_t)(b * H + y) * kW + x0) * NS + lane;
+        out[o] = tot + bv;
+        if (BNP) bt.y[o] = sigmoidf_(tot + bv);
+      }
     }
     __syncthreads();
   }
 }
 
 constexpr int kExpRows = 8;
-template <int CS, int N>
+struct BnBwd {
+  const float *z, *mean, *istd, *gamma, *beta, *slope;
+  double* acc;
+  float* dslope;
+  double* ws;
+  unsigned* ticket;
+};
+
+template <int CS, int N, bool BNR>
 __global__ void __launch_bounds__(256, 1) conv_expand_kernel(const float* __restrict__ in, const float* __restrict__ Wp,
                                                              const float* __restrict__ bias, float* __restrict__ out, int H,
-                                                             int nunits) {
+                                                             int nunits, BnBwd bb) {
+  static_assert(!BNR || N == 128, "the BatchNorm-backward sums map 4 channels to a lane");
   constexpr int RW = (kW + 2) * 4;
   constexpr int ROWF = kW * CS;
   constexpr int NPF = ((kExpRows + 2) * ROWF + 255) / 256;
@@ -192,6 +248,28 @@
   __syncthreads();
   constexpr int STEP = N == 128 ? 2 : 4;
   const int xoff = N == 128 ? 0 : 2 * (lane >> 4);
+  float bm[4], bs[4], bg[4], bt[4], ba = 1.f;
+  double sg[4] = {0, 0, 0, 0}, sgx[4] = {0, 0, 0, 0}, su = 0;
+  if (BNR) {
+#pragma unroll
+    for (int j = 0; j < 4; ++j) {
+      bm[j] = bb.mean[n4 + j];
+      bs[j] = bb.istd[n4 + j];
+      bg[j] = bb.gamma[n4 + j];
+      bt[j] = bb.beta[n4 + j];
+    }
+    ba = *bb.slope;
+  }
+  auto bn_acc = [&](const float4& zv, const float4& dv) {
+    const float z[4] = {zv.x, zv.y, zv.z, zv.w}, d[4] = {dv.x, dv.y, dv.z, dv.w};
+#pragma unroll
+    for (int j = 0; j < 4; ++j) {
+      float xh;
+      const float g = bn_prelu_bwd1(z[j], d[j], bm[j], bs[j], bg[j], bt[j], ba, xh, su);
+      sg[j] += (double)g;
+      sgx[j] += (double)g * (double)xh;
+    }
+  };
   int it = 0;
   for (int unit = blockIdx.x; unit < nunits; unit += gridDim.x, ++it) {
     const int buf = it & 1;
@@ -200,9 +278,24 @@
     const int b = unit / strips, y = (unit - b * strips) * kExpRows + warp;
     const float4* t0 = reinterpret_cast<const float4*>(&tile[buf][warp * RW]);
     float* orow = out + ((size_t)(b * H + y) * kW) * N + n4;
+    const float4* zr = BNR ? reinterpret_cast<const float4*>(bb.z + ((size_t)(b * H + y) * kW) * N + n4) : nullptr;
+    float4 zn0, zn1;
+    if (BNR) {
+      zn0 = zr[0];
+      zn1 = zr[N / 4];
+    }
 #pragma unroll 1
     for (int xb = 0; xb < kW; xb += STEP) {
       const int x = xb + xoff;
+      float4 z0, z1;
+      if (BNR) {
+        z0 = zn0;
+        z1 = zn1;
+        if (xb + STEP < kW) {
+          zn0 = zr[(size_t)(x + STEP) * (N / 4)];
+          zn1 = zr[(size_t)(x + STEP + 1) * (N / 4)];
+        }
+      }
       float4 a0 = b4, a1 = b4;
 #pragma unroll
       for (int dy = 0; dy < 3; ++dy) {
@@ -224,31 +317,72 @@
       }
       *reinterpret_cast<float4*>(orow + (size_t)x * N) = a0;
       *reinterpret_cast<float4*>(orow + (size_t)(x + 1) * N) = a1;
+      if (BNR) {
+        bn_acc(z0, a0);
+        bn_acc(z1, a1);
+      }
     }
     if (more) stash(buf ^ 1);
     __syncthreads();
   }
-}
-
-template <int NS, int VEC>
-int launch_reduce(fg_ctx* c, const float* in, const float* Wp, const float* bias, float* out, const ConvGeom& g) {
+  if (BNR) {
+    __shared__ double red[8][2][N];
+    __shared__ double red_u[8];
+#pragma unroll
+    for (int j = 0; j < 4; ++j) {
+      red[warp][0][n4 + j] = sg[j];
+      red[warp][1][n4 + j] = sgx[j];
+    }
+#pragma unroll
+    for (int o = 16; o > 0; o >>= 1) su += __shfl_xor_sync(0xffffffffu, su, o);
+    if (lane == 0) red_u[warp] = su;
+    __syncthreads();
+    double* row = bb.ws + (int64_t)blockIdx.x * (2 * N + 1);
+    if (threadIdx.x < 2 * N) {
+      const int k = threadIdx.x / N, ch = threadIdx.x % N;
+      double a = 0;
+      for (int wi = 0; wi < 8; ++wi) a += red[wi][k][ch];
+      row[threadIdx.x] = a;
+    }
+    if (threadIdx.x == 0) {
+      double a = 0;
+      for (int wi = 0; wi < 8; ++wi) a += red_u[wi];
+      row[2 * N] = a;
+    }
+    if (ordered_last_block(bb.ticket)) {
+      for (int i = threadIdx.x; i < 2 * N; i += blockDim.x) bb.acc[i] += ordered_sum(bb.ws, gridDim.x, 2 * N + 1, i);
+      if (threadIdx.x == 0) *bb.dslope += (float)ordered_sum(bb.ws, gridDim.x, 2 * N + 1, 2 * N);
+      ordered_release(bb.ticket);
+    }
+  }
+}
+
+template <int NS, int VEC, bool BNP = false>
+int launch_reduce(fg_ctx* c, const float* in, const float* Wp, const float* bias, float* out, const ConvGeom& g,
+                  const BnTail& bt = BnTail{}) {
   CUtensorMap tmap;
   FG_TRY(tc_encode_nhwc_box(&tmap, in, 32 * VEC, g.W, g.H, g.B, 32 * VEC, kW + 2, kRedRows + 2, 1));
   const int nunits = g.B * (g.H / kRedRows);
   const size_t smem = 2 * (size_t)red_tile_bytes<VEC>() + 64 + 128;
   static bool attr_done = false;
   if (!attr_done) {
-    FG_CUDA(cudaFuncSetAttribute(conv_reduce_kernel<NS, VEC>, cudaFuncAttributeMaxDynamicSharedMemorySize, (int)smem));
+    FG_CUDA(cudaFuncSetAttribute(conv_reduce_kernel<NS, VEC, BNP>, cudaFuncAttributeMaxDynamicSharedMemorySize, (int)smem));
     attr_done = true;
   }
-  conv_reduce_kernel<NS, VEC><<<std::min(nunits, c->sm_count), 256, smem, c->stream>>>(tmap, Wp, bias, out, g.H, nunits);
+  conv_reduce_kernel<NS, VEC, BNP><<<std::min(nunits, c->sm_count), 256, smem, c->stream>>>(tmap, Wp, bias, out, g.H, nunits, bt);
   LAUNCH_CHECK(c);
   return FG_OK;
 }
-template <int CS, int N>
-int launch_expand(fg_ctx* c, const float* in, const float* Wp, const float* bias, float* out, const ConvGeom& g) {
+template <int CS, int N, bool BNR = false>
+int launch_expand(fg_ctx* c, const float* in, const float* Wp, const float* bias, float* out, const ConvGeom& g,
+                  const BnBwd& bb = BnBwd{}) {
   const int nunits = g.B * (g.H / kExpRows);
-  conv_expand_kernel<CS, N><<<std::min(nunits, c->sm_count), 256, 0, c->stream>>>(in, Wp, bias, out, g.H, nunits);
+  const int grid = std::min(nunits, c->sm_count);
+  if (BNR) {
+    FG_CUDA(cudaMemsetAsync(bb.acc, 0, sizeof(double) * 2 * N, c->stream));
+    FG_TRY(red_check(c, grid, 2 * N + 1));
+  }
+  conv_expand_kernel<CS, N, BNR><<<grid, 256, 0, c->stream>>>(in, Wp, bias, out, g.H, nunits, bb);
   LAUNCH_CHECK(c);
   return FG_OK;
 }
@@ -279,3 +413,22 @@
   fg_set_error("k_conv_edge: unsupported shape %d -> %d", g.Cin, g.Cout);
   return FG_ERR_UNSUPPORTED;
 }
+
+int k_gen_tail_fwd(fg_ctx* c, const float* z2, const float* mean, const float* istd, const float* gamma, const float* beta,
+                   const float* slope, const float* Wp, const float* bias, float* h, float* z3, float* y, ConvGeom g) {
+  const BnTail bt{mean, istd, gamma, beta, slope, h, y};
+  if (g.Cout == 3 && g.Cin == 128) return launch_reduce<3, 4, true>(c, z2, Wp, bias, z3, g, bt);
+  if (g.Cout == 1 && g.Cin == 128) return launch_reduce<1, 4, true>(c, z2, Wp, bias, z3, g, bt);
+  fg_set_error("k_gen_tail_fwd: unsupported shape %d -> %d", g.Cin, g.Cout);
+  return FG_ERR_UNSUPPORTED;
+}
+
+int k_gen_tail_bwd_reduce(fg_ctx* c, const float* dz3, const float* Wpd, float* dh2, ConvGeom gd, const float* z2,
+                          const float* mean, const float* istd, const float* gamma, const float* beta, const float* slope,
+                          double* acc, float* dslope) {
+  const BnBwd bb{z2, mean, istd, gamma, beta, slope, acc, dslope, c->red_ws, c->red_ticket};
+  if (gd.Cout == 128 && gd.Cin == 3) return launch_expand<3, 128, true>(c, dz3, Wpd, nullptr, dh2, gd, bb);
+  if (gd.Cout == 128 && gd.Cin == 1) return launch_expand<1, 128, true>(c, dz3, Wpd, nullptr, dh2, gd, bb);
+  fg_set_error("k_gen_tail_bwd_reduce: unsupported shape %d -> %d", gd.Cin, gd.Cout);
+  return FG_ERR_UNSUPPORTED;
+}
diff --git a/face_generator_b200/csrc/k_elem.cu b/face_generator_b200/csrc/k_elem.cu
--- a/face_generator_b200/csrc/k_elem.cu
+++ b/face_generator_b200/csrc/k_elem.cu
@@ -1,6 +1,7 @@
 #include <cmath>
 
 #include "fg_internal.h"
+#include "k_act.cuh"
 #include "k_ordered.cuh"
 
 __device__ __forceinline__ int perm_idx(int j, int A, int S) {
@@ -387,16 +388,10 @@
     const float4 g = make_float4(gamma[ch], gamma[ch + 1], gamma[ch + 2], gamma[ch + 3]);
     const float4 b = make_float4(beta[ch], beta[ch + 1], beta[ch + 2], beta[ch + 3]);
     float4 o;
-    o.x = g.x * ((v.x - m.x) * s.x) + b.x;
-    o.y = g.y * ((v.y - m.y) * s.y) + b.y;
-    o.z = g.z * ((v.z - m.z) * s.z) + b.z;
-    o.w = g.w * ((v.w - m.w) * s.w) + b.w;
-    if (act) {
-      o.x = o.x > 0.f ? o.x : a * o.x;
-      o.y = o.y > 0.f ? o.y : a * o.y;
-      o.z = o.z > 0.f ? o.z : a * o.z;
-      o.w = o.w > 0.f ? o.w : a * o.w;
-    }
+    o.x = bn_prelu1(v.x, m.x, s.x, g.x, b.x, act, a);
+    o.y = bn_prelu1(v.y, m.y, s.y, g.y, b.y, act, a);
+    o.z = bn_prelu1(v.z, m.z, s.z, g.z, b.z, act, a);
+    o.w = bn_prelu1(v.w, m.w, s.w, g.w, b.w, act, a);
     if (h) h4[i] = o;
     am = amax4(am, o.x, o.y, o.z, o.w);
     if (hi) {
@@ -420,9 +415,7 @@
   const float a = act ? *slope : 1.f;
   for (int64_t i = blockIdx.x * (int64_t)blockDim.x + threadIdx.x; i < n; i += (int64_t)gridDim.x * blockDim.x) {
     const int ch = (int)(i % C);
-    float o = gamma[ch] * ((z[i] - mean[ch]) * istd[ch]) + beta[ch];
-    if (act) o = o > 0.f ? o : a * o;
-    h[i] = o;
+    h[i] = bn_prelu1(z[i], mean[ch], istd[ch], gamma[ch], beta[ch], act, a);
   }
 }
 int k_bn_prelu_apply(fg_ctx* c, const float* z, const float* mean, const float* istd, const float* gamma,
@@ -649,7 +642,6 @@
   return FG_OK;
 }
 
-__device__ __forceinline__ float sigmoidf_(float x) { return 1.0f / (1.0f + expf(-x)); }
 __global__ void sigmoid_fwd_kernel(const float* __restrict__ z, float* __restrict__ y, int64_t n) {
   for (int64_t i = blockIdx.x * (int64_t)blockDim.x + threadIdx.x; i < n; i += (int64_t)gridDim.x * blockDim.x)
     y[i] = sigmoidf_(z[i]);
diff --git a/face_generator_b200/csrc/nets.cu b/face_generator_b200/csrc/nets.cu
--- a/face_generator_b200/csrc/nets.cu
+++ b/face_generator_b200/csrc/nets.cu
@@ -246,7 +246,7 @@
   const int Bh = B / 2, C = c->C;
   const size_t img = (size_t)C * 1024;
   const float world = (float)c->world;
-  FG_TRY(gen_forward(c->env, c->G, c->net, noiseD, Bh, true));
+  FG_TRY(gen_forward(c->env, c->G, c->net, noiseD, Bh, true, false));
   FG_TRY(k_nchw_to_nhwc(c, real, c->D_x, Bh, C, 1024));
   FG_CUDA(cudaMemcpyAsync(c->D_x + Bh * img, c->G.y, sizeof(float) * Bh * img, cudaMemcpyDeviceToDevice, c->stream));
   if (masksD)
diff --git a/profiles/edge_bytes.py b/profiles/edge_bytes.py
--- /dev/null
+++ b/profiles/edge_bytes.py
@@ -0,0 +1,21 @@
+import sys
+
+B = int(sys.argv[1]) if len(sys.argv) > 1 else 256
+MB = 1e6
+
+
+def act(n, ch):
+    return n * 32 * 32 * ch * 4
+
+
+rows = []
+for step, n, backward in (("D step", B // 2, False), ("G step", B, True)):
+    sep = act(n, 128) * 3 + act(n, 3) * 3
+    fused = act(n, 128) * (2 if backward else 1) + act(n, 3) * 2
+    rows.append((step, n, sep, fused))
+rows.append(("G bwd", B, act(B, 3) + act(B, 128) * 3, act(B, 3) + act(B, 128) * 2))
+for step, n, sep, fused in rows:
+    print("%-7s batch %4d   separate %7.1f MB   fused %7.1f MB" % (step, n, sep / MB, fused / MB))
+tot_sep, tot_fused = sum(r[2] for r in rows), sum(r[3] for r in rows)
+print("step total         separate %7.1f MB   fused %7.1f MB   saved %6.1f MB (%.3f ms at 3 TB/s)" % (
+    tot_sep / MB, tot_fused / MB, (tot_sep - tot_fused) / MB, (tot_sep - tot_fused) / 3e12 * 1e3))
diff --git a/profiles/kernel_times.py b/profiles/kernel_times.py
--- /dev/null
+++ b/profiles/kernel_times.py
@@ -0,0 +1,47 @@
+import json
+import os
+import sys
+from collections import defaultdict
+
+import numpy as np
+import torch
+from torch.profiler import ProfilerActivity, profile
+
+sys.path.insert(0, os.path.dirname(os.path.dirname(os.path.abspath(__file__))))
+import face_generator_b200 as fg
+from face_generator_b200 import layouts as LY
+from face_generator_b200.lib import NET_D, NET_G
+
+B, C = 256, 3
+steps = int(sys.argv[1]) if len(sys.argv) > 1 else 5
+out = sys.argv[2] if len(sys.argv) > 2 else None
+torch.cuda.init()
+rng = np.random.default_rng(1)
+ctx = fg.Context(0, max_batch=B, channels=C)
+ctx.set_option("use_graph", 0)
+for k, v in (a.split("=") for a in sys.argv[3:]):
+    ctx.set_option(k, int(v))
+ctx.set_params(NET_G, LY.trained_like_init(LY.G_layout(C), rng))
+ctx.set_params(NET_D, LY.trained_like_init(LY.D_layout(C), rng, 1.4))
+f = lambda a: np.ascontiguousarray(a, np.float32)
+dev = [ctx.dev_array(f(a)) for a in (rng.random((B // 2, C, 32, 32)), rng.uniform(-1, 1, (B // 2, 100)), rng.uniform(-1, 1, (B, 100)))]
+hyper = fg.hyper_default()
+for i in range(5):
+    ctx.train_step(hyper, B, dev[0], dev[1], dev[2], None, None, i + 1, want_stats=False)
+ctx.sync()
+with profile(activities=[ProfilerActivity.CUDA]) as prof:
+    for i in range(steps):
+        ctx.train_step(hyper, B, dev[0], dev[1], dev[2], None, None, 100 + i, want_stats=False)
+    ctx.sync()
+tot, cnt = defaultdict(float), defaultdict(int)
+for ev in prof.events():
+    if ev.device_type == torch.autograd.DeviceType.CUDA:
+        tot[ev.name] += ev.device_time_total / 1e3 / steps
+        cnt[ev.name] += 1
+rows = sorted(((t, cnt[n] / steps, n) for n, t in tot.items()), reverse=True)
+print("total device ms/step %.4f" % sum(t for t, _, _ in rows))
+for t, n, name in rows:
+    print("%8.4f ms  %5.1f x  %s" % (t, n, name[:160]))
+if out:
+    json.dump([{"ms_per_step": t, "launches_per_step": n, "kernel": name} for t, n, name in rows], open(out, "w"), indent=1)
+ctx.close()
```
